# fy-vision/DiGA

Hardware: AMD Instinct MI355X
Metric: 768x768 19-class crops/sec (DiGA warm-up step) (higher is better)
Workload: dtype f32; 1 GPU; configs[1]: ResNet-101 DeepLabV2 DiGA warm-up (student + EMA teacher, KL distill), synthetic GTA5-shape 768x768, batch 8 per GPU; global_batch=8, parallelism=dp1

## Files before the change

diga_amd/_lib.py:

```python
import collections
import ctypes as C
import os

import torch

from diga_amd import config

_HERE = os.path.dirname(os.path.abspath(__file__))
LIB_PATH = os.environ.get("DIGA_LIB") or os.path.join(_HERE, "libdiga_hip.so")

if not os.path.exists(LIB_PATH):
    raise ImportError(
        f"{LIB_PATH} is missing: the DiGA hot path has no CPU fallback. "
        "Build the HIP extension first: python -m diga_amd.build")

lib = C.CDLL(LIB_PATH)

P = C.c_void_p
I64 = C.c_int64
F32 = C.c_float
INT = C.c_int
SZ = C.c_size_t

SIGNATURES = {
# ... 13 lines not shown
    "diga_ema_update_multi": (INT, [P, P, P, P, P, I64, I64, F32, F32, P]),
    "diga_sgd_momentum_multi": (INT, [P, P, P, P, P, P, P, P, I64, I64, F32, F32, INT, F32, P, P]),
    "diga_nonfinite_flag_f32": (INT, [P, I64, P, P]),
    "diga_label_hist256": (INT, [P, P, I64, I64, P]),
    "diga_classmix_paste": (INT, [P, P, P, P, P, P, P, I64, I64, I64, P]),
    "diga_centroid_softmax_weights": (INT, [P, P, P, P, I64, I64, I64, I64, P]),
    "diga_upsample_argmax_consensus": (INT, [P, P, P, P, I64, I64, I64, I64, I64, I64, P]),
    "diga_class_mean_workspace_bytes": (SZ, [I64, I64]),
    "diga_class_mean_vectors": (INT, [P, P, P, P, P, P, P, SZ, I64, I64, I64, I64, I64, I64, I64, P]),
    "diga_centroid_ema_apply": (INT, [P, P, P, P, I64, I64, I64, I64, F32, INT, INT, P]),
    "diga_confusion_matrix": (INT, [P, P, P, I64, I64, P]),
    "diga_two_scale_confusion": (INT, [P, I64, I64, P, I64, I64, P, P, P, I64, I64, I64, I64, P]),
    "diga_conv2d_nhwc_f32": (INT, [P, P, P, P] + [I64] * 17 + [P, INT, P]),
    "diga_conv2d_nhwc_f32_infer": (INT, [P, P, P, P] + [I64] * 17 + [P, INT, P]),
    "diga_conv2d_stats_floats": (SZ, [I64, I64, I64, I64]),
    "diga_conv2d_stats_chunk_rows": (INT, [I64] * 13 + [INT]),
    "diga_conv2d_epi_chunk_rows": (INT, [I64] * 13 + [INT]),
    "diga_split_bf16": (INT, [P, P, P, I64, P]),
    "diga_conv2d_nhwc_bf16x3": (INT, [P, P, P, P, P] + [I64] * 17 + [P, INT, P]),
    "diga_make_twin": (INT, [P, I64, P, I64, I64, P]),
    "diga_split_bf16_image_bytes": (SZ, [I64, I64, I64]),
    "diga_split_bf16_image": (INT, [P, P, I64, I64, I64, P]),
    "diga_conv2d_nhwc_twin": (INT, [P, P, P, P] + [I64] * 16 + [P, INT, P]),
    "diga_conv2d_nhwc_f32_opts": (INT, [P, P, P, P] + [I64] * 17 + [P, INT, P]),
    "diga_conv2d_nhwc_bf16x3_opts": (INT, [P, P, P, P, P] + [I64] * 17 + [P, INT, P]),
    "diga_conv2d_nhwc_twin_opts": (INT, [P, P, P, P] + [I64] * 16 + [P, INT, P]),
    "diga_conv2d_wgrad_workspace_bytes": (SZ, [I64] * 7),
    "diga_conv2d_wgrad_nhwc_f32": (INT, [P, P, P, P, SZ] + [I64] * 17 + [INT, P]),
    "diga_conv2d_wgrad_twin_workspace_bytes": (SZ, [I64] * 7),
    "diga_conv2d_wgrad_twin": (INT, [P, P, P, P, SZ] + [I64] * 15 + [P]),
    "diga_weight_transpose": (INT, [P, P, I64, I64, I64, P]),
    "diga_dgrad_strided_f32": (INT, [P, I64, P, P] + [I64] * 14 + [P]),
    "diga_make_triplet": (INT, [P, I64, P, I64, I64, P]),
    "diga_split_bf16x6_image_bytes": (SZ, [I64, I64, I64]),
    "diga_split_bf16x6_image": (INT, [P, P, I64, I64, I64, P]),
    "diga_conv2d_nhwc_bf16x6": (INT, [P, P, P, P] + [I64] * 16 + [P, INT, P]),
    "diga_conv2d_nhwc_bf16x6_epi": (INT, [P, P, P] + [I64] * 16 + [P, INT, P]),
    "diga_conv2d_wgrad_bf16x6_workspace_bytes": (SZ, [I64] * 7),
    "diga_conv2d_wgrad_bf16x6": (INT, [P, P, P, P, SZ] + [I64] * 15 + [P]),
    "diga_conv2d_nhwc_bf16x6_f32in": (INT, [P, I64, P, P, P] + [I64] * 16 + [P, INT, P]),
    "diga_conv2d_nhwc_bf16x6_f32in_epi": (INT, [P, I64, P, P] + [I64] * 16 + [P, INT, P]),
    "diga_infer_conv2d_nhwc_bf16x6": (INT, [P, P, P, P] + [I64] * 16 + [P, INT, P]),
    "diga_infer_conv2d_nhwc_bf16x6_f32in": (INT, [P, I64, P, P, P] + [I64] * 16 + [P, INT, P]),
    "diga_conv2d_wgrad_bf16x6_f32in": (INT, [P, I64, P, I64, P, P, SZ] + [I64] * 15 + [P]),
    "diga_conv_taps_bf16x6_f32in": (INT, [P, I64, P, P, P] + [I64] * 16 + [P, INT, P]),
    "diga_conv_taps_bf16x6_f32in_epi": (INT, [P, I64, P, P] + [I64] * 16 + [P, INT, P]),
    "diga_infer_conv_taps_bf16x6_f32in": (INT, [P, I64, P, P, P] + [I64] * 16 + [P, INT, P]),
    "diga_conv_taps_bf16x6_f32in_opts": (INT, [P, I64, P, P, P] + [I64] * 16 + [P, P, INT, P]),
    "diga_conv_window_bf16x6_plan": (INT, [I64] * 9 + [P, P, P]),
    "diga_conv_window_bf16x6_f32in": (INT, [P, I64, P, P, P] + [I64] * 14 + [P, INT, P]),
    "diga_conv_up2_bf16x6_plan": (INT, [I64] * 14 + [P, P]),
    "diga_collapse_up2_weights": (INT, [P, P] + [I64] * 6 + [P]),
    "diga_conv_up2_bf16x6_f32in": (INT, [P, I64, P, P, P, P] + [I64] * 12 + [P, INT, P]),
    "diga_conv_taps_wgrad_bf16x6_workspace_bytes": (SZ, [I64] * 7),
    "diga_conv_taps_wgrad_bf16x6_f32in": (INT, [P, I64, P, I64, P, P, SZ] + [I64] * 15 + [P]),
    "diga_wgrad_bf16x6_tile": (INT, [I64, I64, P, P]),
    "diga_wgrad_bf16x6_tiled_workspace_bytes": (SZ, [I64] * 7),
    "diga_wgrad_bf16x6_tiled_f32in": (INT, [P, I64, P, I64, P, P, SZ] + [I64] * 15 + [P]),
    "diga_im2col_nchw": (INT, [P, P] + [I64] * 11 + [P]),
    "diga_norm_workspace_bytes": (SZ, [I64, I64, I64]),
    "diga_bn_fwd": (INT, [P, I64, P, I64, P, I64, P, P, P, P, P, P, P, I64, I64, INT, INT, INT, P, F32, F32, P, SZ, P]),
    "diga_bn_eval_coefficients": (INT, [P, P, P, P, P, I64, F32, P]),
    "diga_bn_fwd_partials": (INT, [P, I64, P, I64, P, I64, P, P, P, P, P, P, P, I64, I64, INT, INT, P, F32, F32, P, I64, P, SZ, P]),
    "diga_bn_fwd_partials_resab": (INT, [P, I64, P, I64, P, I64, P, P, P, P, P, P, P, I64, I64, P, F32, F32, P, I64, P, SZ, P]),
    "diga_bn_fwd_records": (INT, [P, I64, P, I64, P, I64, P, P, P, P, P, P, P, I64, I64, INT, INT, P, F32, F32, P, P, I64, P, SZ, P]),
    "diga_bn_bwd": (INT, [P, I64, P, I64, P, I64, P, P, P, P, P, I64, P, I64, I64, I64, INT, INT, P, SZ, P]),
    "diga_bn_bwd_affine": (INT, [P, I64, P, I64, P, I64, P, P, P, P, P, I64, P, P, I64, I64, INT, P, SZ, P]),
    "diga_pyramid_sum_fwd": (INT, [P, I64, I64, P, P, I64, I64, P, I64, I64, P, I64, I64, I64, I64, P]),
    "diga_pyramid_sum_bwd": (INT, [P, I64, I64, P, I64, I64, I64, I64, P]),
    "diga_pyramid_sum_fwd3": (INT, [P, I64, I64, P, P, P, P, P, I64, I64, P]),
    "diga_pyramid_sum_bwd3": (INT, [P, I64, I64, P, P, P, I64, I64, P]),
    "diga_bn_bwd_partials": (INT, [P, I64, P, I64, P, P, P, P, I64, I64, I64, INT, P, I64, P, SZ, P]),
    "diga_conv2d_nhwc_f32_epi": (INT, [P, P, P] + [I64] * 17 + [P, INT, P]),
    "diga_conv2d_winograd_workspace_bytes": (SZ, [I64] * 7),
    "diga_conv2d_winograd_tile_table_bytes": (SZ, [I64] * 5),
    "diga_conv2d_winograd_tile_table": (INT, [P] + [I64] * 5 + [P]),
    "diga_conv2d_winograd_stats_records": (SZ, [I64] * 6),
    "diga_conv2d_winograd_stats_floats": (SZ, [I64] * 6),
    "diga_conv2d_winograd_f32": (INT, [P, P, P, P, P, SZ] + [I64] * 9 + [INT, P, P, INT, P]),
    "diga_conv2d_winograd_f32_opts": (INT, [P, P, P, P, P, SZ] + [I64] * 9 + [P, P, INT, P]),
    "diga_conv_winograd_bf16x6_opts": (INT, [P, P, P, P, P, SZ] + [I64] * 9 + [P, P, INT, P]),
    "diga_conv2d_winograd_f32_epi": (INT, [P, P, P, P, SZ] + [I64] * 9 + [INT, P, P, INT, P]),
    "diga_conv2d_winograd_f32_infer": (INT, [P, P, P, P, P, SZ] + [I64] * 9 + [P, P, INT, P]),
    "diga_conv2d_wgrad_winograd_workspace_bytes": (SZ, [I64] * 7 + [INT]),
    "diga_conv2d_wgrad_winograd_f32": (INT, [P, P, P, P, P, SZ] + [I64] * 9 + [P, P]),
    "diga_conv2d_winograd_v_floats": (SZ, [I64] * 6),
    "diga_conv2d_winograd_f32_keep": (INT, [P, P, P, P, P, P, SZ] + [I64] * 9 + [P, P, INT, P]),
    "diga_gemm_batched_bf16x6_f32in": (INT, [P, I64, I64, I64, P, I64, P, P]),
    "diga_wgrad_batched_bf16x6_workspace_bytes": (SZ, [I64] * 4),
    "diga_wgrad_batched_bf16x6_f32in": (INT, [P, P, P, P, SZ] + [I64] * 4 + [P]),
    "diga_conv2d_winograd_bf16x6_workspace_bytes": (SZ, [I64] * 7),
    "diga_conv2d_winograd_bf16x6": (INT, [P, P, P, P, P, P, SZ] + [I64] * 9 + [INT, P, P, P, INT, P]),
    "diga_infer_conv2d_winograd_bf16x6": (INT, [P, P, P, P, P, SZ] + [I64] * 9 + [P, P, INT, P]),
    "diga_conv2d_wgrad_winograd_bf16x6_workspace_bytes": (SZ, [I64] * 7 + [INT]),
    "diga_conv2d_wgrad_winograd_bf16x6": (INT, [P, P, P, P, P, SZ] + [I64] * 9 + [P, P]),
    "diga_conv2d_nhwc_bf16x3_epi": (INT, [P, P, P, P] + [I64] * 17 + [P, INT, P]),
    "diga_conv2d_nhwc_twin_epi": (INT, [P, P, P] + [I64] * 16 + [P, INT, P]),
    "diga_gn_fwd": (INT, [P, I64, P, I64, P, P, P, P, P, I64, I64, I64, I64, INT, F32, P, SZ, P]),
    "diga_gn_bwd": (INT, [P, I64, P, I64, P, I64, P, P, P, P, P, I64, P, P, I64, I64, I64, I64, P, SZ, P]),
    "diga_avgpool_nhwc": (INT, [P, I64, P, I64, I64, I64, P, SZ, P]),
    "diga_colsum_nhwc": (INT, [P, I64, P, I64, I64, P, SZ, P]),
    "diga_small_linear_fwd": (INT, [P, P, P, P, I64, I64, I64, INT, P]),
    "diga_small_linear_bwd": (INT, [P, P, P, P, P, P, P, P, I64, I64, I64, INT, P]),
    "diga_channel_affine": (INT, [P, I64, P, I64, P, P, I64, I64, I64, P]),
    "diga_channel_dot": (INT, [P, I64, P, I64, P, I64, I64, I64, P, SZ, P]),
    "diga_maxpool3x3s2_fwd": (INT, [P, P, P, I64, I64, I64, I64, I64, I64, P]),
    "diga_maxpool3x3s2_bwd": (INT, [P, P, P, I64, I64, I64, I64, I64, I64, P]),
    "diga_color_aug_view": (INT, [P, P, P, P, I64, I64, I64, F32, P, P, P]),
    "diga_ocr_workspace_bytes": (SZ, [I64, I64, I64, I64]),
    "diga_ocr_region_fwd": (INT, [P, I64, P, I64, P, P, I64, I64, I64, I64, P, SZ, P]),
    "diga_ocr_region_bwd": (INT, [P, I64, P, I64, P, P, P, P, I64, P, I64, I64, I64, I64, I64, P]),
    "diga_ocr_attend_fwd": (INT, [P, I64, P, P, P, I64, P, I64, I64, I64, I64, I64, F32, P]),
    "diga_ocr_attend_bwd": (INT, [P, I64, P, P, P, P, I64, P, I64, P, P, I64, I64, I64, I64, I64, F32, P, SZ, P]),
    "diga_mit_gemm_nt": (INT, [P, I64, P, I64, P, P, I64, INT, P, I64, P, I64, INT, F32, I64, I64, I64, P]),
    "diga_mit_gemm_tn_workspace_bytes": (SZ, [I64, I64, I64]),
    "diga_mit_gemm_tn": (INT, [P, I64, P, I64, P, P, F32, INT, P, SZ, I64, I64, I64, P]),
    "diga_mit_colsum_workspace_bytes": (SZ, [I64, I64]),
    "diga_mit_colsum": (INT, [P, I64, P, F32, INT, P, SZ, I64, I64, P]),
    "diga_mit_cast_transpose": (INT, [P, P, P, I64, I64, P]),
    "diga_mit_weight_prep_multi": (INT, [P, P, I64, I64, P]),
    "diga_mit_cast_scale": (INT, [P, P, I64, F32, P]),
    "diga_mit_row_scale": (INT, [P, P, P, I64, I64, I64, P]),
    "diga_mit_layernorm_fwd": (INT, [P, I64, P, P, P, P, I64, P, P, I64, I64, F32, P]),
    "diga_mit_layernorm_bwd_workspace_bytes": (SZ, [I64, I64]),
    "diga_mit_layernorm_bwd": (INT, [P, INT, I64, F32, P, I64, P, P, P, P, I64, P, P, I64, P, P, F32, INT, P, SZ, I64, I64, P]),
    "diga_mit_dwconv_gelu_fwd": (INT, [P, P, P, P, P, I64, I64, I64, I64, P]),
    "diga_mit_dwconv_bwd_workspace_bytes": (SZ, [I64, I64, I64]),
    "diga_mit_dwconv_gelu_bwd": (INT, [P, P, P, P, P, P, P, P, F32, INT, P, SZ, I64, I64, I64, I64, P]),
    "diga_mit_im2col": (INT, [P, INT, P] + [I64] * 11 + [P]),
    "diga_mit_col2im": (INT, [P, P, INT, F32] + [I64] * 11 + [P]),
    "diga_mit_attention_fwd": (INT, [P, I64, P, I64, P, I64, P, I64, I64, I64, I64, F32, P]),
    "diga_mit_attention_bwd_workspace_bytes": (SZ, [I64, I64, I64, I64]),
    "diga_mit_attention_bwd": (INT, [P, I64, P, I64, P, P, I64, P, P, P, P, SZ, I64, I64, I64, I64, F32, P]),
    "diga_prof_enable": (INT, [INT]),
    "diga_prof_reset": (INT, []),
    "diga_prof_query": (INT, [INT, P, P]),
    "diga_prof_query_work": (INT, [INT, P]),
}

class ConvOptions(C.Structure):
    _fields_ = [("reflect_pad", INT), ("upsample_shift", INT), ("activation", INT)]


class MitWeightPrep(C.Structure):
    _fields_ = [("src", P), ("out_a", P), ("out_b", P), ("Co", INT), ("Ci", INT), ("RS", INT), ("Kp", INT), ("mode", INT),
                ("tiles_k", INT)]


class BwdEpilogue(C.Structure):
    _fields_ = [("addend", P), ("addend_ld", I64), ("mask_y", P), ("mask_ld", I64), ("x", P), ("x_ld", I64),
                ("relu_ab", P), ("mean", P), ("invstd", P), ("partials", P), ("mask_bits", P), ("mask_bits_ld", I64)]


class InferEpilogue(C.Structure):
    _fields_ = [("ab", P), ("residual", P), ("residual_ld", I64), ("relu", INT)]


PROF_TAGS = ["ce2d", "distill", "upsample_loss", "ema", "sgd", "classmix_hist", "classmix_paste",
             "centroid_weights", "consensus", "class_means", "centroid_apply", "conv_fwd", "conv_bwd_data",
             "conv_bwd_weight", "norm", "elementwise", "mit_gemm", "mit_wgrad", "mit_attn_fwd", "mit_attn_bwd", "mit_norm",
             "mit_dwconv", "mit_misc"]


def prof_query(tag):
    n, ms = C.c_int64(0), C.c_double(0.0)
    call("diga_prof_query", PROF_TAGS.index(tag), C.byref(n), C.byref(ms))
    return n.value, ms.value

def prof_work(tag):
    w = C.c_double(0.0)
    call("diga_prof_query_work", PROF_TAGS.index(tag), C.byref(w))
    return w.value


for _name, (_res, _args) in SIGNATURES.items():
    _fn = getattr(lib, _name)
    _fn.restype = _res
    _fn.argtypes = _args


CONV_MATH_F32, CONV_MATH_BF16X3, CONV_MATH_BF16X6 = 0, 1, 2


def set_conv_math(mode, exact=None):
    mode = {"f32": 0, "bf16x3": 1, "bf16x6": 2}.get(mode, mode)
    if mode not in (CONV_MATH_F32, CONV_MATH_BF16X3, CONV_MATH_BF16X6):
        raise ValueError(f"conv math must be 0 / 'f32', 1 / 'bf16x3' or 2 / 'bf16x6', not {mode!r}")
    if exact is not None:
        if exact and mode != CONV_MATH_F32:
            raise ValueError("exact=True belongs to the fp32 arithmetic")
        config.active().winograd_max_tile = 2 if exact else config.active().winograd_default_max_tile
    config.active().conv_math = int(mode)


def get_conv_math():
    return config.active().conv_math


def last_error():
    return lib.diga_last_error_string().decode("utf-8", "replace")


def call(name, *args):
    rc = getattr(lib, name)(*args)
    if rc != 0:
        raise RuntimeError(f"{name} failed (code {rc}): {last_error()}")


def stream():
    return C.c_void_p(torch.cuda.current_stream().cuda_stream)


def ptr(t):
    return C.c_void_p(0) if t is None else C.c_void_p(t.data_ptr())


def require_gpu(*tensors):
    for t in tensors:
        if t is not None and not t.is_cuda:
            raise RuntimeError(
                "diga_amd ops run on the GPU only (HIP kernels, no CPU fallback); got a "
                f"{t.device} tensor")


def contiguous(t, dtype=None):
    if t is None:
        return None
    if dtype is not None and t.dtype != dtype:
        t = t.to(dtype)
    return t if t.is_contiguous() else t.contiguous()

# ... 86 lines not shown
```

diga_amd/config.py:

```python
import contextlib
import dataclasses
import os
from dataclasses import dataclass


def _flag(name, default):
    v = os.environ.get(name)
    if v is None:
        return default
    return v not in ("0", "", "false", "False")


@dataclass
class StepConfig:
    teacher_stream: bool = True
    teacher_offset: str = "layer1"
    wgrad_stream: bool = True
    wgrad_hold: int = 4
    wgrad_hold_batch: int = 4
    c4_overlap: int = 2
    c4_overlap_gloo: bool = False
    step_graph: bool = False
    graph_fork_teacher: bool = True
    graph_fork_wgrad: bool = True
    centroid_exchange: str = "allgather"
    conv_math: int = 0
    x6_split: str = "pass"
    x6_winograd: bool = False
    x6_taps: bool = False
    x6_opts: bool = False
    x6_window: bool = False
    x6_up2: bool = False
    x6_wgrad_tile: str = "wide"
    winograd: bool = True
    winograd_ratio: float = 0.62
    winograd_default_max_tile: int = 6
    winograd_max_tile: int = 6
    winograd_keep_v: bool = True
    winograd_stats: bool = True
    keep_v_max_gb: float = 8.0
    keep_v_min_device_gb: float = 160.0
    conv_twin: str = "3"
    twin_only: bool = True
    twin_conv3: str = "1"
    relu_bits: bool = True
    fuse_bwd: bool = True
    junction_chain: bool = True
    fold_downsample_bn: bool = True
    fold_eval_bn: bool = False
    fold_eval_bn_x6: bool = False
    ddp_bucket_mb: int = 25
    ddp_grad_views: bool = True
    ddp_overlap: bool = True
    ddp_single_rank: bool = False
    mit_loss_scale: float = 1024.0

    @classmethod
    def from_env(cls):
        e = os.environ.get
        c = cls()
        c.teacher_stream = _flag("DIGA_TEACHER_STREAM", c.teacher_stream)
        c.teacher_offset = e("DIGA_TEACHER_OFFSET", c.teacher_offset)
        c.wgrad_stream = _flag("DIGA_WGRAD_STREAM", c.wgrad_stream)
        c.wgrad_hold = int(e("DIGA_WGRAD_HOLD", c.wgrad_hold))
        c.wgrad_hold_batch = int(e("DIGA_WGRAD_HOLD_BATCH", c.wgrad_hold_batch))
        c.c4_overlap = int(e("DIGA_C4_OVERLAP", c.c4_overlap))
        c.c4_overlap_gloo = _flag("DIGA_C4_OVERLAP_GLOO", c.c4_overlap_gloo)
        c.step_graph = _flag("DIGA_STEP_GRAPH", c.step_graph)
        c.graph_fork_teacher = _flag("DIGA_GRAPH_FORK_TEACHER", c.graph_fork_teacher)
        c.graph_fork_wgrad = _flag("DIGA_GRAPH_FORK_WGRAD", c.graph_fork_wgrad)
        c.centroid_exchange = e("DIGA_CENTROID_EXCHANGE", c.centroid_exchange)
        c.conv_math = {"bf16x3": 1, "1": 1, "bf16x6": 2, "2": 2}.get(e("DIGA_CONV_MATH", ""), 0)
        c.x6_split = e("DIGA_X6_SPLIT", c.x6_split)
        c.x6_winograd = _flag("DIGA_X6_WINOGRAD", c.x6_winograd)
        c.x6_taps = _flag("DIGA_X6_TAPS", c.x6_taps)
        c.x6_opts = _flag("DIGA_X6_OPTS", c.x6_opts)
        c.x6_window = _flag("DIGA_X6_WINDOW", c.x6_window)
        c.x6_up2 = _flag("DIGA_X6_UP2", c.x6_up2)
        c.x6_wgrad_tile = e("DIGA_X6_WGRAD_TILE", c.x6_wgrad_tile)
        c.winograd = _flag("DIGA_CONV_WINOGRAD", c.winograd)
        c.winograd_ratio = float(e("DIGA_CONV_WINOGRAD_RATIO", c.winograd_ratio))
        c.winograd_default_max_tile = c.winograd_max_tile = int(e("DIGA_CONV_WINOGRAD_TILE", c.winograd_default_max_tile))
        c.winograd_keep_v = _flag("DIGA_WINOGRAD_KEEP_V", c.winograd_keep_v)
        c.winograd_stats = _flag("DIGA_WINOGRAD_STATS", c.winograd_stats)
        c.keep_v_max_gb = float(e("DIGA_WINOGRAD_KEEP_V_MAX_GB", c.keep_v_max_gb))
        c.keep_v_min_device_gb = float(e("DIGA_WINOGRAD_KEEP_V_MIN_DEVICE_GB", c.keep_v_min_device_gb))
        c.conv_twin = e("DIGA_CONV_TWIN", c.conv_twin)
        c.twin_only = _flag("DIGA_TWIN_ONLY", c.twin_only)
        c.twin_conv3 = e("DIGA_TWIN_CONV3", c.twin_conv3)
        c.relu_bits = _flag("DIGA_RELU_BITS", c.relu_bits)
        c.fuse_bwd = _flag("DIGA_FUSE_BWD", c.fuse_bwd)
        c.junction_chain = _flag("DIGA_JUNCTION_CHAIN", c.junction_chain)
        c.fold_downsample_bn = _flag("DIGA_FOLD_DOWNSAMPLE_BN", c.fold_downsample_bn)
        c.fold_eval_bn = _flag("DIGA_FOLD_EVAL_BN", c.fold_eval_bn)
        c.fold_eval_bn_x6 = _flag("DIGA_FOLD_EVAL_BN_X6", c.fold_eval_bn_x6)
        c.ddp_bucket_mb = int(e("DIGA_DDP_BUCKET_MB", c.ddp_bucket_mb))
        c.ddp_grad_views = _flag("DIGA_DDP_GRAD_VIEWS", c.ddp_grad_views)
        c.ddp_overlap = _flag("DIGA_DDP_OVERLAP", c.ddp_overlap)
        c.ddp_single_rank = _flag("DIGA_DDP_SINGLE_RANK", c.ddp_single_rank)
        c.mit_loss_scale = float(e("DIGA_MIT_LOSS_SCALE", c.mit_loss_scale))
        c.validate()
        return c

    def validate(self):
        if self.centroid_exchange not in ("allgather", "allreduce"):
            raise ValueError(f"centroid_exchange must be 'allgather' or 'allreduce', not {self.centroid_exchange!r}")
        if self.c4_overlap not in (0, 1, 2):
            raise ValueError(f"c4_overlap must be 0, 1 or 2, not {self.c4_overlap!r}")
        if self.wgrad_hold < 0:
            raise ValueError(f"wgrad_hold must be >= 0, not {self.wgrad_hold!r}")
        if self.conv_math not in (0, 1, 2):
            raise ValueError(f"conv_math must be 0 (fp32), 1 (split bf16) or 2 (bf16x6), not {self.conv_math!r}")
        if self.x6_split not in ("pass", "loader"):
            raise ValueError(f"x6_split must be 'pass' or 'loader', not {self.x6_split!r}")
        if not isinstance(self.x6_winograd, bool):
            raise ValueError(f"x6_winograd must be a bool, not {self.x6_winograd!r}")
        if not isinstance(self.x6_taps, bool):
            raise ValueError(f"x6_taps must be a bool, not {self.x6_taps!r}")
        if not isinstance(self.x6_opts, bool):
            raise ValueError(f"x6_opts must be a bool, not {self.x6_opts!r}")
        if not isinstance(self.x6_window, bool):
            raise ValueError(f"x6_window must be a bool, not {self.x6_window!r}")
        if not isinstance(self.x6_up2, bool):
            raise ValueError(f"x6_up2 must be a bool, not {self.x6_up2!r}")
        if self.x6_wgrad_tile not in ("wide", "fit"):
            raise ValueError(f"x6_wgrad_tile must be 'wide' or 'fit', not {self.x6_wgrad_tile!r}")
        if not isinstance(self.fold_eval_bn, bool):
            raise ValueError(f"fold_eval_bn must be a bool, not {self.fold_eval_bn!r}")
        if not isinstance(self.fold_eval_bn_x6, bool):
            raise ValueError(f"fold_eval_bn_x6 must be a bool, not {self.fold_eval_bn_x6!r}")
        if self.winograd_max_tile not in (2, 4, 6):
            raise ValueError(f"winograd_max_tile must be 2, 4 or 6, not {self.winograd_max_tile!r}")
        return self

    def replace(self, **fields):
        return dataclasses.replace(self, **fields).validate()

    def serial_streams(self):
        return self.replace(teacher_stream=False, wgrad_stream=False, c4_overlap=0)


DEFAULTS = StepConfig.from_env()
_stack = [DEFAULTS]


def active():
    return _stack[-1]


@contextlib.contextmanager
def use(cfg):
    _stack.append(cfg)
    try:
        yield cfg
    finally:
        _stack.pop()


@contextlib.contextmanager
def override(**fields):
    with use(active().replace(**fields)) as cfg:
        yield cfg
```

diga_amd/csrc/conv.hip:

```cpp
#include <stdlib.h>
#include <string.h>

#include <algorithm>
#include <type_traits>
#include <atomic>

#include "common.h"
#include "conv_call.h"

namespace diga {

using f32x16 = __attribute__((ext_vector_type(16))) float;
using f32x4nt = __attribute__((ext_vector_type(4))) float;

__device__ __forceinline__ void store4_stream(float* p, float x, float y, float z, float w) {
#if defined(DIGA_PROBE_NOSTORE)
    if (x == 1.2345e38f) *p = y + z + w;
#elif defined(DIGA_PROBE_PLAINSTORE)
    *reinterpret_cast<float4*>(p) = make_float4(x, y, z, w);
#else
    __builtin_nontemporal_store((f32x4nt){x, y, z, w}, reinterpret_cast<f32x4nt*>(p));
#endif
}

constexpr int kBK = 32;

struct ConvArgs {
    const float* in;
    const float* wgt;
    const uint16_t* wgt_hi;
    const uint16_t* wgt_lo;
    const unsigned char* wgt_img;
    const float* bias;
    float* out;
    float* stats;
    int N, Hi, Wi, Cin, in_ld;
    int Ho, Wo, Cout, out_ld;
    int R, S, sy, sx;
    int oy0, ox0, ody, odx;
    int M, tiles_m, tiles_n;
    int all_inside;
    const float* e_add;
    const float* e_masky;
    const unsigned char* e_maskbits;
    const float* e_x;
    const float* e_relu_ab;
    const float* e_mean;
    const float* e_invstd;
    float* e_partials;
    int e_add_ld, e_masky_ld, e_x_ld, e_maskbits_ld;
    int pad_reflect;
    int up_shift;
    int act;
    int wb_tiles = 0;
    int64_t wb_stride = 0;
    const float* i_ab = nullptr;
    const float* i_res = nullptr;
    int i_res_ld = 0;
    int i_relu = 0;
};

__device__ __forceinline__ bool map_tap(const ConvArgs& a, int iy, int ix, int& py, int& px) {
    const int Hl = a.Hi << a.up_shift, Wl = a.Wi << a.up_shift;
    bool ok = (unsigned)iy < (unsigned)Hl && (unsigned)ix < (unsigned)Wl;
    if (a.pad_reflect) {
        iy = iy < 0 ? -iy : (iy >= Hl ? 2 * (Hl - 1) - iy : iy);
        ix = ix < 0 ? -ix : (ix >= Wl ? 2 * (Wl - 1) - ix : ix);
        ok = true;
    }
    py = min(max(iy, 0), Hl - 1) >> a.up_shift;
    px = min(max(ix, 0), Wl - 1) >> a.up_shift;
    return ok;
}

__device__ __forceinline__ int xcd_remap(int orig, int nwg) {
    const int xcd = orig & 7, q = nwg >> 3, r = nwg & 7;
    return (xcd < r ? xcd * (q + 1) : r * (q + 1) + (xcd - r) * q) + (orig >> 3);
}

template <int TM, int TN, bool EPI = false, int NTHR = 256, bool INF = false, int TAG = 0>
__device__ __forceinline__ void drain_stage(const float* stage_in, const ConvArgs& a, int m0, int n0, int t, int tile_m,
                                            bool active = true);

template <int TM, int TN, bool EPI = false, bool INF = false>
__device__ __forceinline__ void epilogue_tile(f32x16 (&acc)[TM][TN], float* __restrict__ stage, const ConvArgs& a,
                                              int m0, int n0, int wm, int wn, int lane, int t, int tile_m) {
    constexpr int BN = 64 * TN, LDS_LD = BN + 4;
    const int li = lane & 31, lh = lane >> 5;
#pragma unroll
    for (int j = 0; j < TN; ++j)
#pragma unroll
// ... 2020 lines not shown
            nx = nx == 2 ? 0 : nx + 1;
        }
        return;
    }

    const int wm = wv >> 1, wn = wv & 1;
    f32x16 acc[2][2];
#pragma unroll
    for (int i = 0; i < 2; ++i)
#pragma unroll
        for (int j = 0; j < 2; ++j)
#pragma unroll
            for (int e = 0; e < 16; ++e) acc[i][j][e] = 0.f;
    const int li = lane & 31, lh = lane >> 5;
    int offa[2], offb[2];
#pragma unroll
    for (int i = 0; i < 2; ++i) {
        offa[i] = lh * A_ROW + (((wm * 64 + i * 32 + li) * 4) ^ (lh << 7));
        offb[i] = A_BYTES + lh * B_ROW + (((wn * 64 + i * 32 + li) * 4) ^ (lh << 7));
    }

    __builtin_amdgcn_s_barrier();
    int cur = 0;
    for (int ks = 0; ks < ksteps; ++ks) {
        const unsigned char* St = smem_b + cur * STAGE;
        float av[2][2], bv[2][2];
        auto frag = [&](int kk, int set) {
#pragma unroll
            for (int i = 0; i < 2; ++i) av[set][i] = *reinterpret_cast<const float*>(St + offa[i] + kk * A_ROW);
#pragma unroll
            for (int j = 0; j < 2; ++j) bv[set][j] = *reinterpret_cast<const float*>(St + offb[j] + kk * B_ROW);
        };
        frag(0, 0);
#pragma unroll
        for (int kk = 0; kk < kBK; kk += 2) {
            const int set = (kk >> 1) & 1;
            if (kk + 2 < kBK) frag(kk + 2, set ^ 1);
            __builtin_amdgcn_sched_group_barrier(0x100, 4, 0);
#pragma unroll
            for (int i = 0; i < 2; ++i)
#pragma unroll
                for (int j = 0; j < 2; ++j)
                    acc[i][j] = __builtin_amdgcn_mfma_f32_32x32x2f32(av[set][i], bv[set][j], acc[i][j], 0, 0, 0);
            __builtin_amdgcn_sched_group_barrier(0x008, 4, 0);
        }
        asm volatile("s_waitcnt lgkmcnt(0)" ::: "memory");
        __builtin_amdgcn_s_barrier();
        cur = cur == 2 ? 0 : cur + 1;
    }

    float* out = a.slab + (int64_t)split * a.Cout * RS * a.Cin;
#pragma unroll
    for (int j = 0; j < 2; ++j) {
        const int c = c0 + wn * 64 + j * 32 + li;
#pragma unroll
        for (int i = 0; i < 2; ++i) {
#pragma unroll
            for (int e = 0; e < 16; ++e) {
                const int k = k0 + wm * 64 + i * 32 + (e & 3) + 8 * (e >> 2) + 4 * lh;
                out[((int64_t)k * RS + tap) * a.Cin + c] = acc[i][j][e];
            }
        }
    }
}

__global__ __launch_bounds__(256) void slab_reduce_kernel(const float* __restrict__ slab, float* __restrict__ dw,
                                                          int64_t n4, int splits) {
    const int64_t i = (int64_t)blockIdx.x * 256 + threadIdx.x;
    if (i >= n4) return;
    float4 s = reinterpret_cast<const float4*>(slab)[i];
    for (int k = 1; k < splits; ++k) {
        const float4 v = reinterpret_cast<const float4*>(slab)[(int64_t)k * n4 + i];
        s.x += v.x;
        s.y += v.y;
        s.z += v.z;
        s.w += v.w;
    }
    reinterpret_cast<float4*>(dw)[i] = s;
}

__global__ __launch_bounds__(256) void weight_transpose_kernel(const float* __restrict__ w, float* __restrict__ wt,
                                                               int K, int RS, int C) {
    __shared__ float tile[32][33];
    const int tap = blockIdx.z;
    const int k0 = blockIdx.y * 32, c0 = blockIdx.x * 32;
    const int tx = threadIdx.x & 31, ty = threadIdx.x >> 5;
#pragma unroll
    for (int i = 0; i < 4; ++i) {
        const int k = k0 + ty + 8 * i, c = c0 + tx;
        tile[ty + 8 * i][tx] = (k < K && c < C) ? w[((int64_t)k * RS + tap) * C + c] : 0.f;
    }
    __syncthreads();
#pragma unroll
    for (int i = 0; i < 4; ++i) {
        const int c = c0 + ty + 8 * i, k = k0 + tx;
        if (c < C && k < K) wt[((int64_t)c * RS + tap) * K + k] = tile[tx][ty + 8 * i];
    }
}

static int check_conv_common(const char* who, int64_t Cin, int64_t in_ld, int64_t out_ld, int64_t Cout,
                             const void* in, const void* w, const void* out) {
    DIGA_REQUIRE(Cin > 0 && Cin % 32 == 0, DIGA_EINVAL, "%s: Cin=%lld must be a multiple of 32", who, (long long)Cin);
    DIGA_REQUIRE(in_ld >= Cin && in_ld % 4 == 0 && out_ld >= Cout, DIGA_EINVAL, "%s: bad leading dimensions", who);
    DIGA_REQUIRE(aligned16(in) && aligned16(w), DIGA_EALIGN, "%s: pointers must be 16-byte aligned", who);
    (void)out;
    return DIGA_OK;
}

static int check_options(const diga_conv_options_t* o, const char* who) {
    if (o == nullptr) return DIGA_OK;
    DIGA_REQUIRE(o->reflect_pad >= 0 && o->reflect_pad <= 1 && o->upsample_shift >= 0 && o->upsample_shift <= 2 && o->activation >= 0 &&
                     o->activation <= 1, DIGA_EINVAL, "%s: bad options (reflect_pad 0/1, upsample_shift 0..2, activation 0/1)", who);
    return DIGA_OK;
}

static int fill_conv_args(ConvArgs& a, const ConvCall& c, const char* who, const char* who_infer) {
    a = ConvArgs{};
    a.in = static_cast<const float*>(c.in); a.wgt = c.wgt; a.wgt_hi = c.wgt_hi; a.wgt_lo = c.wgt_lo;
    a.wgt_img = static_cast<const unsigned char*>(c.wgt_img); a.bias = c.bias; a.out = c.out; a.stats = c.stats;
    a.N = (int)c.N; a.Hi = (int)c.Hi; a.Wi = (int)c.Wi; a.Cin = (int)c.Cin; a.in_ld = (int)(c.in_ld >= 0 ? c.in_ld : c.Cin);
    a.Ho = (int)c.Ho; a.Wo = (int)c.Wo; a.Cout = (int)c.Cout; a.out_ld = (int)c.out_ld;
    a.R = (int)c.R; a.S = (int)c.S; a.sy = (int)c.stride_y; a.sx = (int)c.stride_x;
    a.oy0 = (int)c.off_y0; a.ox0 = (int)c.off_x0; a.ody = (int)c.off_dy; a.odx = (int)c.off_dx;
    a.M = (int)(c.N * c.Ho * c.Wo);
    int rc = check_options(c.opts, who);
    if (rc) return rc;
    if (const diga_conv_options_t* o = c.opts) {
        a.pad_reflect = o->reflect_pad; a.up_shift = o->upsample_shift; a.act = o->activation;
    }
    const bool out4 = c.Cout % 4 == 0 && c.out_ld % 4 == 0 && aligned16(c.out) && c.stats == nullptr;
    rc = check_bwd_epilogue(c.epi, c.Cout, who, out4 && c.bias == nullptr);
    if (rc) return rc;
    if (const diga_bwd_epilogue_t* e = c.epi) {
        a.e_add = e->addend; a.e_add_ld = (int)e->addend_ld;
        a.e_masky = e->mask_y; a.e_masky_ld = (int)e->mask_ld;
        a.e_maskbits = e->mask_bits; a.e_maskbits_ld = (int)e->mask_bits_ld;
        a.e_x = e->x; a.e_x_ld = (int)e->x_ld;
        a.e_relu_ab = e->relu_ab; a.e_mean = e->mean; a.e_invstd = e->invstd; a.e_partials = e->partials;
    }
    rc = check_infer_epilogue(c.infer, c.Cout, c.out, who_infer, out4 && (c.bias == nullptr || aligned16(c.bias)));
    if (rc) return rc;
    if (const diga_infer_epilogue_t* e = c.infer) {
        a.i_ab = e->ab;
        a.i_res = e->residual;
        a.i_res_ld = e->residual ? (int)e->residual_ld : 0;
        a.i_relu = e->relu ? 1 : 0;
    }
    return DIGA_OK;
}

template <class Args>
static void launch_k(void (*kernel)(Args), unsigned grid, unsigned threads, size_t sh, hipStream_t st, const Args& a) {
    (void)hipFuncSetAttribute((const void*)kernel, hipFuncAttributeMaxDynamicSharedMemorySize, (int)sh);
    hipLaunchKernelGGL(kernel, dim3(grid), dim3(threads), sh, st, a);
}
using ConvKernel = void (*)(ConvArgs);
using WgradKernel = void (*)(WgradArgs);

struct GemmArgs {
    const float* A;
    const float* W;
    float* out;
    int M, K, Cout, tiles_m, tiles_n, wb_tiles;
    int rows_valid;
    int64_t wb_stride;
    int64_t a_ld, out_ld;
    const float* bias;
    float* stats;
    const float* i_ab = nullptr;
    const float* i_res = nullptr;
    int64_t i_res_ld = 0;
    int i_relu = 0;
};

template <bool STATS, bool BIAS, int INF = 0>
__global__ __launch_bounds__(768, 3) void gemm_f32_persistent_kernel(GemmArgs g) {
    static_assert(INF == 0 || !STATS, "no statistics next to the inference epilogue");
    constexpr int A_BYTES = 256 * 128, B_BYTES = 128 * 128, STAGE = A_BYTES + B_BYTES;
    extern __shared__ __align__(16) unsigned char smem_b[];
    const int lane = threadIdx.x & 63, wv = threadIdx.x >> 6;
// ... 868 lines not shown
```

diga_amd/csrc/winograd.hip:

```cpp
#include <type_traits>

#include "common.h"
#include "conv_call.h"

namespace diga {

int gemm_batched_f32_dma(const float* A, int64_t rows_per_batch, int batches, int64_t K, const float* W, int64_t Cout,
                         float* out, hipStream_t st, int64_t rows_valid);
size_t wgrad_batched_slab_bytes(int64_t rows, int batches, int64_t Cout, int64_t Cin);
int wgrad_batched_f32_dma(const float* Z, const float* V, float* dU, float* slab, int64_t rows, int batches, int64_t Cout,
                          int64_t Cin, hipStream_t st);
int split_image3_batched(const float* U, void* imgs, int batches, int64_t Cout, int64_t K, hipStream_t st);
bool gemm_batched_bf16x6_ok(int64_t rows_per_batch, int64_t batches, int64_t K, int64_t Cout);
int gemm_batched_bf16x6(const float* A, int64_t rows_per_batch, int batches, int64_t K, const void* imgs, int64_t Cout, float* out,
                        hipStream_t st);
bool wgrad_batched_bf16x6_ok(int64_t rows, int64_t batches, int64_t Cout, int64_t Cin);
size_t wgrad_batched_bf16x6_slab_bytes(int64_t rows, int batches, int64_t Cout, int64_t Cin);
int wgrad_batched_bf16x6(const float* Z, const float* V, float* dU, float* slab, int64_t rows, int batches, int64_t Cout, int64_t Cin,
                         hipStream_t st);

namespace wino {

struct WinoGeom {
    int N, H, W, d;
    int m;
    int tys, txs;
    int64_t T, Tp;
};

int phase_tiles(int len, int d, int m) {
    int s = 0;
    for (int a = 0; a < d; ++a) {
        const int n = len > a ? (len - a + d - 1) / d : 0;
        s += (n + m - 1) / m;
    }
    return s;
}

WinoGeom make_wino(int64_t N, int64_t H, int64_t W, int64_t d, int64_t m) {
    WinoGeom g;
    g.N = (int)N; g.H = (int)H; g.W = (int)W; g.d = (int)d; g.m = (int)m;
    g.tys = phase_tiles((int)H, (int)d, (int)m);
    g.txs = phase_tiles((int)W, (int)d, (int)m);
    g.T = N * g.tys * g.txs;
    g.Tp = ceil_div(g.T, 256) * 256;
    return g;
}
static inline int products(int64_t m) { return (int)((m + 2) * (m + 2)); }
static inline bool tile_ok(int64_t m) { return m == 2 || m == 4 || m == 6; }

__global__ __launch_bounds__(256) void wino_tiles_kernel(int4* __restrict__ tab, WinoGeom g) {
    const int64_t t = (int64_t)blockIdx.x * 256 + threadIdx.x;
    if (t >= g.Tp) return;
    if (t >= g.T) {
        tab[t] = make_int4(-1, 0, 0, 0);
        return;
    }
    const int timg = g.tys * g.txs;
    const int n = (int)(t / timg), r = (int)(t - (int64_t)n * timg);
    constexpr int kBand = 1;
    const int band = r / (kBand * g.txs), rem = r - band * kBand * g.txs;
    const int rows_in_band = min(kBand, g.tys - kBand * band);
    int Cc = rem / rows_in_band, R = kBand * band + (rem - Cc * rows_in_band);
    int a = 0, b = 0;
    for (; a < g.d; ++a) {
        const int cnt = g.H > a ? (g.H - a + g.d - 1) / g.d : 0;
        const int tl = (cnt + g.m - 1) / g.m;
        if (R < tl) break;
        R -= tl;
    }
    for (; b < g.d; ++b) {
        const int cnt = g.W > b ? (g.W - b + g.d - 1) / g.d : 0;
        const int tl = (cnt + g.m - 1) / g.m;
        if (Cc < tl) break;
        Cc -= tl;
    }
    tab[t] = make_int4(n, a + g.m * R * g.d, b + g.m * Cc * g.d, 0);
}

using f32x4nt = __attribute__((ext_vector_type(4))) float;
__device__ __forceinline__ void nt_store4(float* p, float4 v) {
    __builtin_nontemporal_store((f32x4nt){v.x, v.y, v.z, v.w}, reinterpret_cast<f32x4nt*>(p));
}
__device__ __forceinline__ float4 nt_load4(const float* p) {
    const f32x4nt v = __builtin_nontemporal_load(reinterpret_cast<const f32x4nt*>(p));
    return make_float4(v.x, v.y, v.z, v.w);
// ... 4 lines not shown

__device__ __forceinline__ float4 f4fma(float s, float4 a, float4 b) {
    return make_float4(__builtin_fmaf(s, a.x, b.x), __builtin_fmaf(s, a.y, b.y), __builtin_fmaf(s, a.z, b.z), __builtin_fmaf(s, a.w, b.w));
}
__device__ __forceinline__ float4 f4scale(float s, float4 a) { return make_float4(s * a.x, s * a.y, s * a.z, s * a.w); }
__device__ __forceinline__ float2 f4add(float2 a, float2 b) { return make_float2(a.x + b.x, a.y + b.y); }
__device__ __forceinline__ float2 f4sub(float2 a, float2 b) { return make_float2(a.x - b.x, a.y - b.y); }
__device__ __forceinline__ float2 f4fma(float s, float2 a, float2 b) { return make_float2(__builtin_fmaf(s, a.x, b.x), __builtin_fmaf(s, a.y, b.y)); }
__device__ __forceinline__ float2 f4scale(float s, float2 a) { return make_float2(s * a.x, s * a.y); }
__device__ __forceinline__ float f4add(float a, float b) { return a + b; }
__device__ __forceinline__ float f4sub(float a, float b) { return a - b; }
__device__ __forceinline__ float f4fma(float s, float a, float b) { return __builtin_fmaf(s, a, b); }
__device__ __forceinline__ float f4scale(float s, float a) { return s * a; }
__device__ __forceinline__ void nt_store4(float* p, float v) { __builtin_nontemporal_store(v, p); }
using f32x2nt = __attribute__((ext_vector_type(2))) float;
__device__ __forceinline__ void nt_store4(float* p, float2 v) {
    __builtin_nontemporal_store((f32x2nt){v.x, v.y}, reinterpret_cast<f32x2nt*>(p));
}
template <typename V> __device__ __forceinline__ V nt_loadv(const float* p);
template <> __device__ __forceinline__ float4 nt_loadv<float4>(const float* p) { return nt_load4(p); }
template <> __device__ __forceinline__ float2 nt_loadv<float2>(const float* p) {
    const f32x2nt v = __builtin_nontemporal_load(reinterpret_cast<const f32x2nt*>(p));
    return make_float2(v.x, v.y);
}
template <> __device__ __forceinline__ float nt_loadv<float>(const float* p) { return __builtin_nontemporal_load(p); }
template <typename V> __device__ __forceinline__ V vzero();
template <> __device__ __forceinline__ float vzero<float>() { return 0.f; }
template <> __device__ __forceinline__ float4 vzero<float4>() { return make_float4(0.f, 0.f, 0.f, 0.f); }
template <> __device__ __forceinline__ float2 vzero<float2>() { return make_float2(0.f, 0.f); }

#include "winograd_xforms.h"

template <int M> struct Xf;
template <> struct Xf<2> {
    template <typename V> static __device__ __forceinline__ void bt(const V* x, V* r) {
        r[0] = f4sub(x[0], x[2]);
        r[1] = f4add(x[1], x[2]);
        r[2] = f4sub(x[2], x[1]);
        r[3] = f4sub(x[1], x[3]);
    }
    template <typename V> static __device__ __forceinline__ void g(const V* x, V* r) {
        const V sum = f4add(x[0], x[2]);
        r[0] = x[0];
        r[1] = f4half(f4add(sum, x[1]));
        r[2] = f4half(f4sub(sum, x[1]));
        r[3] = x[2];
    }
    template <typename V> static __device__ __forceinline__ void at(const V* x, V* r) {
        r[0] = f4add(f4add(x[0], x[1]), x[2]);
        r[1] = f4sub(f4sub(x[1], x[2]), x[3]);
    }
    template <typename V> static __device__ __forceinline__ void a(const V* x, V* r) {
        r[0] = x[0];
        r[1] = f4add(x[0], x[1]);
        r[2] = f4sub(x[0], x[1]);
        r[3] = f4sub(vzero<V>(), x[1]);
    }
    template <typename V> static __device__ __forceinline__ void gt(const V* x, V* r) {
        const V hs = f4half(f4add(x[1], x[2])), hd = f4half(f4sub(x[1], x[2]));
        r[0] = f4add(x[0], hs);
        r[1] = hd;
        r[2] = f4add(hs, x[3]);
    }
};
template <> struct Xf<4> {
    template <typename V> static __device__ __forceinline__ void bt(const V* x, V* r) { wino4_bt(x, r); }
    template <typename V> static __device__ __forceinline__ void g(const V* x, V* r) { wino4_g(x, r); }
    template <typename V> static __device__ __forceinline__ void at(const V* x, V* r) { wino4_at(x, r); }
    template <typename V> static __device__ __forceinline__ void a(const V* x, V* r) { wino4_a(x, r); }
    template <typename V> static __device__ __forceinline__ void gt(const V* x, V* r) { wino4_gt(x, r); }
};
template <> struct Xf<6> {
    template <typename V> static __device__ __forceinline__ void bt(const V* x, V* r) { wino6_bt(x, r); }
    template <typename V> static __device__ __forceinline__ void g(const V* x, V* r) { wino6_g(x, r); }
    template <typename V> static __device__ __forceinline__ void at(const V* x, V* r) { wino6_at(x, r); }
    template <typename V> static __device__ __forceinline__ void a(const V* x, V* r) { wino6_a(x, r); }
    template <typename V> static __device__ __forceinline__ void gt(const V* x, V* r) { wino6_gt(x, r); }
};
template <int M> struct Vec;
template <> struct Vec<2> { using In = float4; using Out = float4; using Dy = float4; using Dw = float4; static constexpr int EpiLanes = 4, EpiBlocks = 3; };
template <> struct Vec<4> { using In = float4; using Out = float2; using Dy = float4; using Dw = float2; static constexpr int EpiLanes = 2, EpiBlocks = 4; };
template <> struct Vec<6> { using In = float2; using Out = float; using Dy = float2; using Dw = float2; static constexpr int EpiLanes = 2, EpiBlocks = 4; };

template <int M>
__global__ __launch_bounds__(256) void winoM_weight_kernel(const float* __restrict__ w, float* __restrict__ U, int Cout, int Cin,
                                                           int flip) {
    constexpr int A = M + 2;
    const int64_t idx = (int64_t)blockIdx.x * 256 + threadIdx.x;
    const int c4n = Cin / 4;
    if (idx >= (int64_t)Cout * c4n) return;
    const int co = (int)(idx / c4n), c = (int)(idx - (int64_t)co * c4n) * 4;
    float4 t[A][3];
#pragma unroll
    for (int s = 0; s < 3; ++s) {
        float4 g[3];
#pragma unroll
        for (int r = 0; r < 3; ++r) {
            const int rr = flip ? 2 - r : r, ss = flip ? 2 - s : s;
            g[r] = *reinterpret_cast<const float4*>(w + ((int64_t)co * 9 + rr * 3 + ss) * Cin + c);
        }
        float4 col[A];
        Xf<M>::g(g, col);
#pragma unroll
        for (int i = 0; i < A; ++i) t[i][s] = col[i];
    }
    const int64_t plane = (int64_t)Cout * Cin;
    float* o = U + (int64_t)co * Cin + c;
#pragma unroll
    for (int i = 0; i < A; ++i) {
        float4 row[A];
        Xf<M>::g(t[i], row);
#pragma unroll
        for (int j = 0; j < A; ++j) *reinterpret_cast<float4*>(o + (A * i + j) * plane) = row[j];
    }
}

template <typename V> __device__ __forceinline__ void wino_in_store(float* p, V v) { nt_store4(p, v); }
template <int M, typename V, bool REFLECT = false>
__global__ __launch_bounds__(256) void winoM_input_kernel(const float* __restrict__ x, int64_t ld, const int4* __restrict__ tab,
                                                          float* __restrict__ Vo, int64_t Tp, int C, int H, int W, int d) {
    constexpr bool reflect = REFLECT;
    constexpr int A = M + 2;
    constexpr int VW = sizeof(V) / 4;
    const int c4n = C / VW;
    const int64_t idx = (int64_t)blockIdx.x * 256 + threadIdx.x;
    if (idx >= Tp * c4n) return;
    const int64_t t = idx / c4n;
    const int c = (int)(idx - t * c4n) * VW;
    const int4 e = tab[t];
    const V z = vzero<V>();
    const int img = max(e.x, 0);
    V m[A][A];
#pragma unroll
    for (int j = 0; j < A; ++j) {
        int xx = e.z + (j - 1) * d;
        if (reflect) {
            xx = xx < 0 ? -xx : xx;
            xx = xx >= W ? 2 * (W - 1) - xx : xx;
        }
        const bool xok = e.x >= 0 && (reflect || (unsigned)xx < (unsigned)W);
        const int xc = min(max(xx, 0), W - 1);
        V p[A];
#pragma unroll
        for (int i = 0; i < A; ++i) {
            int y = e.y + (i - 1) * d;
            if (reflect) {
                y = y < 0 ? -y : y;
                y = y >= H ? 2 * (H - 1) - y : y;
            }
            const bool ok = xok && (reflect || (unsigned)y < (unsigned)H);
            const int yc = min(max(y, 0), H - 1);
            const V v = *reinterpret_cast<const V*>(x + ((int64_t)(img * H + yc) * W + xc) * ld + c);
            p[i] = ok ? v : z;
        }
        V col[A];
        Xf<M>::bt(p, col);
#pragma unroll
        for (int i = 0; i < A; ++i) m[i][j] = col[i];
    }
    float* o = Vo + t * C + c;
    const int64_t plane = Tp * C;
#pragma unroll
    for (int i = 0; i < A; ++i) {
        V row[A];
        Xf<M>::bt(m[i], row);
#pragma unroll
        for (int j = 0; j < A; ++j) wino_in_store<V>(o + (A * i + j) * plane, row[j]);
    }
}

__global__ __launch_bounds__(256) void wino_input_kernel(const float* __restrict__ x, int64_t ld, const int4* __restrict__ tab,
                                                         float* __restrict__ V, int64_t Tp, int C, int H, int W, int d) {
    const int c4n = C / 4;
    const int64_t idx = (int64_t)blockIdx.x * 256 + threadIdx.x;
    if (idx >= Tp * c4n) return;
    const int64_t t = idx / c4n;
    const int c = (int)(idx - t * c4n) * 4;
    const int4 e = tab[t];
    const float4 z = make_float4(0.f, 0.f, 0.f, 0.f);
    const int img = max(e.x, 0);
    float4 p[4][4];
#pragma unroll
    for (int i = 0; i < 4; ++i) {
        const int y = e.y + (i - 1) * d;
        const bool yok = e.x >= 0 && (unsigned)y < (unsigned)H;
        const int yc = min(max(y, 0), H - 1);
#pragma unroll
        for (int j = 0; j < 4; ++j) {
            const int xx = e.z + (j - 1) * d;
            const bool ok = yok && (unsigned)xx < (unsigned)W;
            const float4 v = *reinterpret_cast<const float4*>(x + ((int64_t)(img * H + yc) * W + min(max(xx, 0), W - 1)) * ld + c);
            p[i][j] = ok ? v : z;
        }
    }
    float4 m[4][4];
#pragma unroll
// ... 459 lines not shown
                           (int)Cout, g.H, g.W, g.d, tpb, ep);
}
template <int M, bool ADD>
static void launch_output_epi2_mask(const float* Mb, const int4* tab, float* out, int64_t out_ld, const WinoGeom& g, int64_t Cout, int64_t G,
                                    int tpb, const WinoEpi& ep, hipStream_t st) {
    if (ep.masky != nullptr) launch_output_epi2_sums<M, ADD, 1>(Mb, tab, out, out_ld, g, Cout, G, tpb, ep, st);
    else if (ep.maskbits != nullptr) launch_output_epi2_sums<M, ADD, 2>(Mb, tab, out, out_ld, g, Cout, G, tpb, ep, st);
    else if (ep.relu_ab != nullptr) launch_output_epi2_sums<M, ADD, 3>(Mb, tab, out, out_ld, g, Cout, G, tpb, ep, st);
    else launch_output_epi2_sums<M, ADD, 0>(Mb, tab, out, out_ld, g, Cout, G, tpb, ep, st);
}
template <int M>
static void launch_output_epi2_m(const float* Mb, const int4* tab, float* out, int64_t out_ld, const WinoGeom& g, int64_t Cout, int64_t G,
                                 int tpb, const WinoEpi& ep, hipStream_t st) {
    if (ep.add != nullptr) launch_output_epi2_mask<M, true>(Mb, tab, out, out_ld, g, Cout, G, tpb, ep, st);
    else launch_output_epi2_mask<M, false>(Mb, tab, out, out_ld, g, Cout, G, tpb, ep, st);
}

template <int M>
static void launch_dy_m(const float* dy, int64_t dy_ld, const int4* tab, float* Z, const WinoGeom& g, int64_t Cout, hipStream_t st) {
    using VT = typename Vec<M>::Dy;
    constexpr int VW = sizeof(VT) / 4;
    hipLaunchKernelGGL((winoM_dy_kernel<M, VT>), dim3((unsigned)ceil_div(g.Tp * (Cout / VW), 256)), dim3(256), 0, st, dy, dy_ld, tab, Z, g.Tp,
                       (int)Cout, g.H, g.W, g.d);
}
template <int M>
static void launch_dw_m(const float* dU, float* dw, int64_t Cout, int64_t Cin, hipStream_t st) {
    using VT = typename Vec<M>::Dw;
    constexpr int VW = sizeof(VT) / 4;
    hipLaunchKernelGGL((winoM_dw_kernel<M, VT>), dim3((unsigned)ceil_div(Cout * (Cin / VW), 256)), dim3(256), 0, st, dU, dw, (int)Cout, (int)Cin);
}

struct WinoWgradLayout {
    size_t tab, V, Z, dU, slab, total;
};
WinoWgradLayout wino_wgrad_layout(const WinoGeom& g, int64_t Cin, int64_t Cout, bool with_v, bool x6 = false) {
    WinoWgradLayout l;
    size_t o = 0;
    l.tab = o; o += (size_t)g.Tp * sizeof(int4);
    l.V = o; o += with_v ? (size_t)products(g.m) * g.Tp * Cin * sizeof(float) : 0;
    l.Z = o; o += (size_t)products(g.m) * g.Tp * Cout * sizeof(float);
    l.dU = o; o += (size_t)products(g.m) * Cout * Cin * sizeof(float);
    l.slab = o; o += x6 ? wgrad_batched_bf16x6_slab_bytes(g.Tp, products(g.m), Cout, Cin)
                        : wgrad_batched_slab_bytes(g.Tp, products(g.m), Cout, Cin);
    l.total = o + 64;
    return l;
}

struct WinoLayout {
    size_t tab, U, img, V, M, total;
};
WinoLayout wino_layout(const WinoGeom& g, int64_t Cin, int64_t Cout, bool x6 = false) {
    WinoLayout l;
    size_t o = 0;
    l.tab = o; o += (size_t)g.Tp * sizeof(int4);
    l.U = o; o += (size_t)products(g.m) * Cout * Cin * sizeof(float);
    l.img = o; o += x6 ? (size_t)products(g.m) * diga_split_bf16x6_image_bytes(Cout, 1, Cin) : 0;
    l.V = o; o += (size_t)products(g.m) * g.Tp * Cin * sizeof(float);
    l.M = o; o += (size_t)products(g.m) * g.Tp * Cout * sizeof(float);
    l.total = o + 64;
    return l;
}

struct WinoShape {
    void* workspace = nullptr;
    size_t workspace_bytes = 0;
    int64_t N = 0, H = 0, W = 0, Cin = 0, Cout = 0, dilation = 0, tile = 0;
    const void* tile_table = nullptr;
    void* stream = nullptr;
    bool x6 = false;
};
#define DIGA_FILL_WINO(c_)                                                                                              \
    do {                                                                                                               \
        (c_).workspace = workspace; (c_).workspace_bytes = workspace_bytes; (c_).N = N; (c_).H = H; (c_).W = W; (c_).Cin = Cin;     \
        (c_).Cout = Cout; (c_).dilation = dilation; (c_).tile = tile; (c_).tile_table = tile_table; (c_).stream = stream;          \
    } while (0)
struct WinoCall : WinoShape {
    const float* in = nullptr;
    const float* wgt = nullptr;
    const float* bias = nullptr;
    float* out = nullptr;
    int64_t in_ld = 0, out_ld = 0;
    int flip = 0, reflect = 0, prof_tag = 0;
    float* v_keep = nullptr;
    float* stats = nullptr;
    const diga_bwd_epilogue_t* epi = nullptr;
    const diga_infer_epilogue_t* infer = nullptr;
};
struct WinoWgradCall : WinoShape {
    const float* dy = nullptr;
    const float* x = nullptr;
    const float* v_kept = nullptr;
    float* dw = nullptr;
    int64_t x_ld = 0, dy_ld = 0;
};

}
}

using namespace diga;
using namespace diga::wino;

extern "C" size_t diga_conv2d_winograd_workspace_bytes(int64_t N, int64_t H, int64_t W, int64_t Cin, int64_t Cout, int64_t dilation, int64_t tile) {
    if (N <= 0 || H <= 0 || W <= 0 || Cin <= 0 || Cout <= 0 || dilation <= 0 || !tile_ok(tile)) return 0;
    return wino_layout(make_wino(N, H, W, dilation, tile), Cin, Cout).total;
}

static int winograd_conv(const WinoCall& c) {
    const float *in = c.in, *wgt = c.wgt, *bias = c.bias;
    float *out = c.out, *stats = c.stats;
    const int64_t N = c.N, H = c.H, W = c.W, Cin = c.Cin, in_ld = c.in_ld, Cout = c.Cout, out_ld = c.out_ld, dilation = c.dilation, tile = c.tile;
    const int flip = c.flip, reflect = c.reflect;
    const bool x6 = c.x6;
    const diga_bwd_epilogue_t* epi = c.epi;
    const diga_infer_epilogue_t* inf = c.infer;
    const void* tile_table = c.tile_table;
    DIGA_REQUIRE(!inf || ((tile == 4 || tile == 6) && !flip && !epi && !stats && !reflect), DIGA_EINVAL,
                 "conv2d_winograd_infer: the inference epilogue comes with the plain forward of 4x4 / 6x6 tiles");
    DIGA_REQUIRE(!reflect || (tile != 2 && !flip && !epi && dilation < H && dilation < W), DIGA_EINVAL,
                 "conv2d_winograd: reflection padding comes with the forward of 4x4 / 6x6 tiles (pad < H, W)");
    DIGA_REQUIRE(in && wgt && out && c.workspace, DIGA_EINVAL, "conv2d_winograd: null pointer");
    DIGA_REQUIRE(N > 0 && H > 0 && W > 0 && dilation > 0 && dilation < 4096, DIGA_EINVAL, "conv2d_winograd: bad shape");
    DIGA_REQUIRE(tile_ok(tile), DIGA_EINVAL, "conv2d_winograd: tile must be 2, 4 or 6 (F(2x2,3x3) / F(4x4,3x3) / F(6x6,3x3))");
    DIGA_REQUIRE(Cin % 32 == 0 && Cout % 4 == 0 && Cout > 64 && in_ld >= Cin && in_ld % 4 == 0 && out_ld >= Cout && out_ld % 4 == 0,
                 DIGA_EINVAL, "conv2d_winograd: Cin %% 32, Cout %% 4 (> 64) and leading dimensions %% 4 required");
    DIGA_REQUIRE(aligned16(in) && aligned16(wgt) && aligned16(out) && aligned16(c.workspace) && (!bias || aligned16(bias)), DIGA_EALIGN,
                 "conv2d_winograd: pointers must be 16-byte aligned");
    DIGA_REQUIRE(N * H * W < (1ll << 31), DIGA_EINVAL, "conv2d_winograd: too many pixels");
    const WinoGeom g = make_wino(N, H, W, dilation, tile);
    const int P = products(tile);
    DIGA_REQUIRE(x6 || P * g.Tp / 256 < 32768, DIGA_EINVAL, "conv2d_winograd: too many tiles for one launch");
    DIGA_REQUIRE(!x6 || gemm_batched_bf16x6_ok(g.Tp, P, Cin, Cout), DIGA_EINVAL,
                 "conv2d_winograd_bf16x6: products * padded tiles and the GEMM's tile count must stay below 2^31");
    const WinoLayout l = wino_layout(g, Cin, Cout, x6);
    DIGA_REQUIRE(c.workspace_bytes >= l.total, DIGA_EWORKSPACE, "conv2d_winograd: workspace too small (%zu < %zu)", c.workspace_bytes, l.total);
    DIGA_REQUIRE(!stats || (epi == nullptr && tile != 2 && aligned16(stats)), DIGA_EINVAL,
                 "conv2d_winograd: statistics come with the forward output transform of 4x4 / 6x6 tiles (16-byte aligned buffer)");
    DIGA_REQUIRE(!tile_table || aligned16(tile_table), DIGA_EALIGN, "conv2d_winograd: tile_table must be 16-byte aligned");
    char* ws = static_cast<char*>(c.workspace);
    const int4* tab = tile_table != nullptr ? static_cast<const int4*>(tile_table) : reinterpret_cast<const int4*>(ws + l.tab);
    float* U = reinterpret_cast<float*>(ws + l.U);
    float* V = c.v_keep != nullptr ? c.v_keep : reinterpret_cast<float*>(ws + l.V);
    float* Mb = reinterpret_cast<float*>(ws + l.M);
    hipStream_t st = (hipStream_t)c.stream;
    ProfScope prof(c.prof_tag == DIGA_PROF_CONV_BWD_DATA ? DIGA_PROF_CONV_BWD_DATA : DIGA_PROF_CONV_FWD, st,
                   2.0 * (double)(N * H * W) * (double)Cout * 9.0 * (double)Cin);
    if (tile_table == nullptr)
        hipLaunchKernelGGL(wino_tiles_kernel, dim3((unsigned)ceil_div(g.Tp, 256)), dim3(256), 0, st, reinterpret_cast<int4*>(ws + l.tab), g);
    with_tile(tile, [&](auto m) { launch_weight_m<decltype(m)::value>(wgt, U, Cout, Cin, flip, st); });
    launch_input(tile, in, in_ld, tab, V, g.Tp, Cin, H, W, dilation, st, reflect);
    int rc;
    if (x6) {
        void* imgs = ws + l.img;
        split_image3_batched(U, imgs, P, Cout, Cin, st);
        rc = gemm_batched_bf16x6(V, g.Tp, P, Cin, imgs, Cout, Mb, st);
    } else {
        rc = gemm_batched_f32_dma(V, g.Tp, P, Cin, U, Cout, Mb, st, g.T);
    }
    if (rc) return rc;
    if (epi == nullptr && stats != nullptr) {
        with_tile<4>(tile, [&](auto m) { launch_output_stats_m<decltype(m)::value>(Mb, tab, bias, out, out_ld, g, Cout, stats, st); });
    } else if (epi == nullptr && inf != nullptr) {
        with_tile<4>(tile, [&](auto m) { launch_output_infer_m<decltype(m)::value>(Mb, tab, bias, out, out_ld, g, Cout, *inf, st); });
    } else if (epi == nullptr) {
        with_tile(tile, [&](auto m) { launch_output_m<decltype(m)::value>(Mb, tab, bias, out, out_ld, g, Cout, st); });
    } else {
        WinoEpi ep;
        ep.add = epi->addend; ep.add_ld = epi->addend_ld;
        ep.masky = epi->mask_y; ep.masky_ld = epi->mask_ld;
        ep.maskbits = epi->mask_bits; ep.maskbits_ld = epi->mask_bits_ld;
        ep.x = epi->x; ep.x_ld = epi->x_ld;
        ep.relu_ab = epi->relu_ab; ep.mean = epi->mean; ep.invstd = epi->invstd; ep.partials = epi->partials;
        const int64_t G = ceil_div(N * H * W, 128);
        const int tpb = (int)ceil_div(g.T, G);
        with_tile(tile, [&](auto m) { launch_output_epi2_m<decltype(m)::value>(Mb, tab, out, out_ld, g, Cout, G, tpb, ep, st); });
    }
    return launch_status(x6 ? (reflect ? "diga_conv_winograd_bf16x6_opts" : "diga_conv2d_winograd_bf16x6") : "diga_conv2d_winograd_f32");
}

extern "C" size_t diga_conv2d_winograd_tile_table_bytes(int64_t N, int64_t H, int64_t W, int64_t dilation, int64_t tile) {
    if (N <= 0 || H <= 0 || W <= 0 || dilation <= 0 || !tile_ok(tile)) return 0;
    return (size_t)make_wino(N, H, W, dilation, tile).Tp * sizeof(int4);
}

extern "C" int diga_conv2d_winograd_tile_table(void* table, int64_t N, int64_t H, int64_t W, int64_t dilation, int64_t tile, void* stream) {
    DIGA_REQUIRE(table && aligned16(table), DIGA_EINVAL, "conv2d_winograd_tile_table: null / unaligned table");
    DIGA_REQUIRE(N > 0 && H > 0 && W > 0 && dilation > 0 && dilation < 4096 && tile_ok(tile) && N * H * W < (1ll << 31), DIGA_EINVAL,
                 "conv2d_winograd_tile_table: bad shape / tile");
    const WinoGeom g = make_wino(N, H, W, dilation, tile);
    hipLaunchKernelGGL(wino_tiles_kernel, dim3((unsigned)ceil_div(g.Tp, 256)), dim3(256), 0, (hipStream_t)stream, static_cast<int4*>(table), g);
    return launch_status("diga_conv2d_winograd_tile_table");
}

extern "C" size_t diga_conv2d_winograd_stats_records(int64_t N, int64_t H, int64_t W, int64_t Cout, int64_t dilation, int64_t tile) {
    if (N <= 0 || H <= 0 || W <= 0 || Cout <= 0 || dilation <= 0 || (tile != 4 && tile != 6)) return 0;
    return (size_t)stats_plan(make_wino(N, H, W, dilation, tile), Cout).records;
}

extern "C" size_t diga_conv2d_winograd_stats_floats(int64_t N, int64_t H, int64_t W, int64_t Cout, int64_t dilation, int64_t tile) {
    const size_t r = diga_conv2d_winograd_stats_records(N, H, W, Cout, dilation, tile);
    return r * 3 * (size_t)Cout + r;
}

extern "C" int diga_conv2d_winograd_f32(const float* in, const float* wgt, const float* bias, float* out, void* workspace,
                                        size_t workspace_bytes, int64_t N, int64_t H, int64_t W, int64_t Cin, int64_t in_ld,
                                        int64_t Cout, int64_t out_ld, int64_t dilation, int64_t tile, int flip, float* stats_partial,
                                        const void* tile_table, int prof_tag, void* stream) {
    WinoCall c;
    DIGA_FILL_WINO(c);
    c.in = in; c.in_ld = in_ld; c.wgt = wgt; c.bias = bias; c.out = out; c.out_ld = out_ld; c.flip = flip; c.stats = stats_partial;
    c.prof_tag = prof_tag;
    return winograd_conv(c);
}

extern "C" int diga_conv2d_winograd_f32_opts(const float* in, const float* wgt, const float* bias, float* out, void* workspace,
                                             size_t workspace_bytes, int64_t N, int64_t H, int64_t W, int64_t Cin, int64_t in_ld,
                                             int64_t Cout, int64_t out_ld, int64_t dilation, int64_t tile, const diga_conv_options_t* opts,
                                             const void* tile_table, int prof_tag, void* stream) {
    DIGA_REQUIRE(opts != nullptr, DIGA_EINVAL, "conv2d_winograd_opts: null options");
    DIGA_REQUIRE(opts->upsample_shift == 0 && opts->activation == 0, DIGA_EINVAL,
                 "conv2d_winograd_opts: only reflect_pad is folded on the Winograd path (upsampling / tanh: the direct `_opts` kernels)");
    WinoCall c;
    DIGA_FILL_WINO(c);
    c.in = in; c.in_ld = in_ld; c.wgt = wgt; c.bias = bias; c.out = out; c.out_ld = out_ld; c.reflect = opts->reflect_pad ? 1 : 0;
    c.prof_tag = prof_tag;
    return winograd_conv(c);
}

extern "C" int diga_conv2d_winograd_f32_infer(const float* in, const float* wgt, const float* bias, float* out, void* workspace,
                                              size_t workspace_bytes, int64_t N, int64_t H, int64_t W, int64_t Cin, int64_t in_ld,
                                              int64_t Cout, int64_t out_ld, int64_t dilation, int64_t tile,
                                              const diga_infer_epilogue_t* infer, const void* tile_table, int prof_tag, void* stream) {
    DIGA_REQUIRE(infer != nullptr, DIGA_EINVAL, "conv2d_winograd_infer: null epilogue descriptor");
    const int rc = check_infer_epilogue(infer, Cout, out, "conv2d_winograd_infer");
    if (rc) return rc;
    WinoCall c;
    DIGA_FILL_WINO(c);
    c.in = in; c.in_ld = in_ld; c.wgt = wgt; c.bias = bias; c.out = out; c.out_ld = out_ld; c.infer = infer; c.prof_tag = prof_tag;
    return winograd_conv(c);
}

extern "C" size_t diga_conv2d_winograd_v_floats(int64_t N, int64_t H, int64_t W, int64_t Cin, int64_t dilation, int64_t tile) {
    if (N <= 0 || H <= 0 || W <= 0 || Cin <= 0 || dilation <= 0 || !tile_ok(tile)) return 0;
    return (size_t)products(tile) * make_wino(N, H, W, dilation, tile).Tp * Cin;
}

extern "C" int diga_conv2d_winograd_f32_keep(const float* in, const float* wgt, const float* bias, float* out, float* v_keep,
                                             void* workspace, size_t workspace_bytes, int64_t N, int64_t H, int64_t W, int64_t Cin,
                                             int64_t in_ld, int64_t Cout, int64_t out_ld, int64_t dilation, int64_t tile,
                                             float* stats_partial, const void* tile_table, int prof_tag, void* stream) {
    DIGA_REQUIRE(v_keep != nullptr && aligned16(v_keep), DIGA_EINVAL, "conv2d_winograd_keep: v_keep must be a 16-byte aligned buffer");
    WinoCall c;
    DIGA_FILL_WINO(c);
    c.in = in; c.in_ld = in_ld; c.wgt = wgt; c.bias = bias; c.out = out; c.out_ld = out_ld; c.v_keep = v_keep; c.stats = stats_partial;
    c.prof_tag = prof_tag;
    return winograd_conv(c);
}

extern "C" int diga_conv2d_winograd_f32_epi(const float* in, const float* wgt, float* out, void* workspace, size_t workspace_bytes,
                                            int64_t N, int64_t H, int64_t W, int64_t Cin, int64_t in_ld, int64_t Cout,
                                            int64_t out_ld, int64_t dilation, int64_t tile, int flip, const diga_bwd_epilogue_t* e,
                                            const void* tile_table, int prof_tag, void* stream) {
    DIGA_REQUIRE(e != nullptr, DIGA_EINVAL, "conv2d_winograd_epi: null epilogue descriptor");
    const int rc = check_bwd_epilogue(e, Cout, "conv2d_winograd_epi");
    if (rc) return rc;
    WinoCall c;
    DIGA_FILL_WINO(c);
    c.in = in; c.in_ld = in_ld; c.wgt = wgt; c.out = out; c.out_ld = out_ld; c.flip = flip; c.epi = e; c.prof_tag = prof_tag;
    return winograd_conv(c);
}

extern "C" size_t diga_conv2d_wgrad_winograd_workspace_bytes(int64_t N, int64_t H, int64_t W, int64_t Cin, int64_t Cout,
                                                             int64_t dilation, int64_t tile, int v_kept) {
    if (N <= 0 || H <= 0 || W <= 0 || Cin <= 0 || Cout <= 0 || dilation <= 0 || Cout % 256 != 0 || Cin % 128 != 0 || !tile_ok(tile)) return 0;
    return wino_wgrad_layout(make_wino(N, H, W, dilation, tile), Cin, Cout, v_kept == 0).total;
}

static int winograd_wgrad(const WinoWgradCall& c) {
    const float *dy = c.dy, *x = c.x, *v_kept = c.v_kept;
    float* dw = c.dw;
    void* workspace = c.workspace;
    const int64_t N = c.N, H = c.H, W = c.W, Cin = c.Cin, x_ld = c.x_ld, Cout = c.Cout, dy_ld = c.dy_ld, dilation = c.dilation, tile = c.tile;
    const void* tile_table = c.tile_table;
    const bool x6 = c.x6;
    DIGA_REQUIRE(!tile_table || aligned16(tile_table), DIGA_EALIGN, "conv2d_wgrad_winograd: tile_table must be 16-byte aligned");
    DIGA_REQUIRE(dy && (x || v_kept) && dw && workspace, DIGA_EINVAL, "conv2d_wgrad_winograd: null pointer");
    DIGA_REQUIRE(!v_kept || aligned16(v_kept), DIGA_EALIGN, "conv2d_wgrad_winograd: v_kept must be 16-byte aligned");
    DIGA_REQUIRE(N > 0 && H > 0 && W > 0 && dilation > 0 && dilation < 4096 && N * H * W < (1ll << 31) && tile_ok(tile),
                 DIGA_EINVAL, "conv2d_wgrad_winograd: bad shape / tile");
    DIGA_REQUIRE(Cout % 256 == 0 && Cin % 128 == 0 && x_ld >= Cin && x_ld % 4 == 0 && dy_ld >= Cout && dy_ld % 4 == 0, DIGA_EINVAL,
                 "conv2d_wgrad_winograd: Cout %% 256, Cin %% 128 and leading dimensions %% 4 required");
    DIGA_REQUIRE(aligned16(dy) && (!x || aligned16(x)) && aligned16(dw) && aligned16(workspace), DIGA_EALIGN,
                 "conv2d_wgrad_winograd: pointers must be 16-byte aligned");
    const WinoGeom g = make_wino(N, H, W, dilation, tile);
    DIGA_REQUIRE(!x6 || wgrad_batched_bf16x6_ok(g.Tp, products(tile), Cout, Cin), DIGA_EINVAL,
                 "conv2d_wgrad_winograd_bf16x6: padded tiles and the GEMM's block count must stay below 2^31");
    const WinoWgradLayout l = wino_wgrad_layout(g, Cin, Cout, v_kept == nullptr, x6);
    DIGA_REQUIRE(c.workspace_bytes >= l.total, DIGA_EWORKSPACE, "conv2d_wgrad_winograd: workspace too small (%zu < %zu)", c.workspace_bytes,
                 l.total);
    char* ws = static_cast<char*>(workspace);
    const int4* tab = tile_table != nullptr ? static_cast<const int4*>(tile_table) : reinterpret_cast<const int4*>(ws + l.tab);
    const float* V = v_kept != nullptr ? v_kept : reinterpret_cast<float*>(ws + l.V);
    float* Z = reinterpret_cast<float*>(ws + l.Z);
    float* dU = reinterpret_cast<float*>(ws + l.dU);
    float* slab = reinterpret_cast<float*>(ws + l.slab);
    hipStream_t st = (hipStream_t)c.stream;
    ProfScope prof(DIGA_PROF_CONV_BWD_WEIGHT, st, 2.0 * (double)(N * H * W) * (double)Cout * 9.0 * (double)Cin);
    if (tile_table == nullptr)
        hipLaunchKernelGGL(wino_tiles_kernel, dim3((unsigned)ceil_div(g.Tp, 256)), dim3(256), 0, st, reinterpret_cast<int4*>(ws + l.tab), g);
    if (v_kept == nullptr)
        launch_input(tile, x, x_ld, tab, reinterpret_cast<float*>(ws + l.V), g.Tp, Cin, H, W, dilation, st);
    with_tile(tile, [&](auto m) { launch_dy_m<decltype(m)::value>(dy, dy_ld, tab, Z, g, Cout, st); });
    int rc = x6 ? wgrad_batched_bf16x6(Z, V, dU, slab, g.Tp, products(tile), Cout, Cin, st)
                : wgrad_batched_f32_dma(Z, V, dU, slab, g.Tp, products(tile), Cout, Cin, st);
    if (rc) return rc;
    with_tile(tile, [&](auto m) { launch_dw_m<decltype(m)::value>(dU, dw, Cout, Cin, st); });
    return launch_status(x6 ? "diga_conv2d_wgrad_winograd_bf16x6" : "diga_conv2d_wgrad_winograd_f32");
}

extern "C" int diga_conv2d_wgrad_winograd_f32(const float* dy, const float* x, const float* v_kept, float* dw, void* workspace,
                                              size_t workspace_bytes, int64_t N, int64_t H, int64_t W, int64_t Cin, int64_t x_ld,
                                              int64_t Cout, int64_t dy_ld, int64_t dilation, int64_t tile, const void* tile_table,
                                              void* stream) {
    WinoWgradCall c;
    DIGA_FILL_WINO(c);
    c.dy = dy; c.dy_ld = dy_ld; c.x = x; c.x_ld = x_ld; c.v_kept = v_kept; c.dw = dw;
    return winograd_wgrad(c);
}

extern "C" size_t diga_conv2d_winograd_bf16x6_workspace_bytes(int64_t N, int64_t H, int64_t W, int64_t Cin, int64_t Cout,
                                                              int64_t dilation, int64_t tile) {
    if (N <= 0 || H <= 0 || W <= 0 || Cin <= 0 || Cin % 32 != 0 || Cout <= 64 || Cout % 4 != 0 || dilation <= 0 || dilation >= 4096 ||
        !tile_ok(tile) || N * H * W >= (1ll << 31))
        return 0;
    const WinoGeom g = make_wino(N, H, W, dilation, tile);
    if (!gemm_batched_bf16x6_ok(g.Tp, products(tile), Cin, Cout)) return 0;
    return wino_layout(g, Cin, Cout, true).total;
}

extern "C" int diga_conv2d_winograd_bf16x6(const float* in, const float* wgt, const float* bias, float* out, float* v_keep,
                                           void* workspace, size_t workspace_bytes, int64_t N, int64_t H, int64_t W, int64_t Cin,
                                           int64_t in_ld, int64_t Cout, int64_t out_ld, int64_t dilation, int64_t tile, int flip,
                                           float* stats_partial, const diga_bwd_epilogue_t* e, const void* tile_table, int prof_tag,
                                           void* stream) {
    DIGA_REQUIRE(!v_keep || aligned16(v_keep), DIGA_EALIGN, "conv2d_winograd_bf16x6: v_keep must be 16-byte aligned");
    DIGA_REQUIRE(!v_keep || (!flip && !e), DIGA_EINVAL, "conv2d_winograd_bf16x6: v_keep comes with the forward (flip = 0, no epilogue)");
    DIGA_REQUIRE(!e || (!bias && !stats_partial), DIGA_EINVAL, "conv2d_winograd_bf16x6: a backward epilogue takes no bias and no statistics");
    const int rc = check_bwd_epilogue(e, Cout, "conv2d_winograd_bf16x6");
    if (rc) return rc;
    WinoCall c;
    DIGA_FILL_WINO(c);
// ... 53 lines not shown
```

diga_amd/model/conv.py:

```python
import ctypes
import os
import sys
from typing import NamedTuple

import torch
import torch.nn as nn

_pkg = os.path.dirname(os.path.dirname(os.path.abspath(__file__)))
if os.path.dirname(_pkg) not in sys.path:
    sys.path.append(os.path.dirname(_pkg))
from diga_amd import _lib, config

_TAG_FWD, _TAG_BWD_DATA = _lib.PROF_TAGS.index("conv_fwd"), _lib.PROF_TAGS.index("conv_bwd_data")


def _pad_to(c, q=32):
    return (c + q - 1) // q * q


def _pad_last(t, c_to):
    c = t.shape[-1]
    if c == c_to:
        return t
    out = t.new_zeros(t.shape[:-1] + (c_to,))
    out[..., :c] = t
    return out



def _bias_grad(gy):
    k = gy.shape[-1]
    ld = gy.stride(2)
    m = gy.shape[0] * gy.shape[1] * gy.shape[2]
    dense = gy.stride(3) == 1 and gy.stride(1) == gy.shape[2] * ld and gy.stride(0) == gy.shape[1] * gy.stride(1)
    if not dense or ((k % 4 != 0 or ld % 4 != 0) and k > 64):
        return gy.sum(dim=(0, 1, 2))
    out = torch.empty(k, dtype=torch.float32, device=gy.device)
    ws = _lib.workspace(_lib.lib.diga_norm_workspace_bytes(m, 1, k), gy.device, "norm")
    _lib.call("diga_colsum_nhwc", _lib.ptr(gy), ld, _lib.ptr(out), m, k, _lib.ptr(ws), ws.numel(), _lib.stream())
    return out


def _use_twin(cin, k, taps, shared):
    mode = config.active().conv_twin
    if mode == "0" or cin % 32 != 0 or k <= 64:
        return False
    return mode == "1" or taps > 1 or shared


def _use_x6(cin, r, s):
    return r == 1 and s == 1 and cin % 32 == 0


def _x6_taps():
    return _lib.get_conv_math() == 2 and config.active().x6_taps


def _x6_opts():
    return _lib.get_conv_math() == 2 and config.active().x6_opts


def _taps_ok(cin, r, s, copt):
    return 1 < r * s <= 64 and cin % 32 == 0 and (not copt or _x6_opts())


def _x6_window(hi, wi, cin, k, r, s, doff, shift):
    if not (_x6_taps() and config.active().x6_window) or doff[0] < 1 or doff[1] < 1:
        return False
    th, tw, cols = ctypes.c_int(0), ctypes.c_int(0), ctypes.c_int(0)
    return _lib.lib.diga_conv_window_bf16x6_plan(hi, wi, cin, k, r, s, doff[0], doff[1], shift, ctypes.byref(th), ctypes.byref(tw),
                                                 ctypes.byref(cols)) == 1


def _x6_up2(hi, wi, cin, k, ho, wo, r, s, off0, doff, opts):
    if not (_x6_opts() and config.active().x6_up2):
        return False
    rc, sc = ctypes.c_int(0), ctypes.c_int(0)
    return _lib.lib.diga_conv_up2_bf16x6_plan(hi, wi, cin, k, ho, wo, r, s, off0[0], off0[1], doff[0], doff[1], int(opts[1]),
                                              int(opts[0]), ctypes.byref(rc), ctypes.byref(sc)) == 1


def _x6_fit(kp, cp):
    if _lib.get_conv_math() != 2 or config.active().x6_wgrad_tile != "fit":
        return False
    bm, bn = ctypes.c_int(0), ctypes.c_int(0)
    _lib.call("diga_wgrad_bf16x6_tile", kp, cp, ctypes.byref(bm), ctypes.byref(bn))
    return (bm.value, bn.value) != (256, 128)


def _x6_loader():
    return config.active().x6_split == "loader"


def _nhwc_ld(t):
# ... 254 lines not shown
            ld = rn.shape[3]
        e.residual, e.residual_ld = _lib.ptr(rn), ld
    e.relu = 1 if relu else 0
    return e, (ab, rn)


def _make_split(src, ld, rows, ch, triplet):
    out = torch.empty(rows * ch * (6 if triplet else 4), dtype=torch.uint8, device=src.device)
    _lib.call("diga_make_triplet" if triplet else "diga_make_twin", _lib.ptr(src), ld, _lib.ptr(out), rows, ch, _lib.stream())
    return out


_ENTRY = {
    ("x6ls", ""): "diga_conv2d_nhwc_bf16x6_f32in", ("x6ls", "epi"): "diga_conv2d_nhwc_bf16x6_f32in_epi",
    ("x6ls", "infer"): "diga_infer_conv2d_nhwc_bf16x6_f32in",
    ("x6rs", ""): "diga_conv_taps_bf16x6_f32in", ("x6rs", "epi"): "diga_conv_taps_bf16x6_f32in_epi",
    ("x6rs", "infer"): "diga_infer_conv_taps_bf16x6_f32in", ("x6rs", "opts"): "diga_conv_taps_bf16x6_f32in_opts",
    ("x6win", ""): "diga_conv_window_bf16x6_f32in", ("x6win", "opts"): "diga_conv_window_bf16x6_f32in",
    ("x6up2", "opts"): "diga_conv_up2_bf16x6_f32in",
    ("x6", ""): "diga_conv2d_nhwc_bf16x6", ("x6", "epi"): "diga_conv2d_nhwc_bf16x6_epi", ("x6", "infer"): "diga_infer_conv2d_nhwc_bf16x6",
    ("twin", ""): "diga_conv2d_nhwc_twin", ("twin", "epi"): "diga_conv2d_nhwc_twin_epi", ("twin", "opts"): "diga_conv2d_nhwc_twin_opts",
    ("bf16x3", ""): "diga_conv2d_nhwc_bf16x3", ("bf16x3", "epi"): "diga_conv2d_nhwc_bf16x3_epi",
    ("bf16x3", "opts"): "diga_conv2d_nhwc_bf16x3_opts",
    ("f32", ""): "diga_conv2d_nhwc_f32", ("f32", "epi"): "diga_conv2d_nhwc_f32_epi", ("f32", "opts"): "diga_conv2d_nhwc_f32_opts",
    ("f32", "infer"): "diga_conv2d_nhwc_f32_infer",
    ("winograd", ""): "diga_conv2d_winograd_f32", ("winograd", "epi"): "diga_conv2d_winograd_f32_epi",
    ("winograd", "infer"): "diga_conv2d_winograd_f32_infer", ("winograd", "keep"): "diga_conv2d_winograd_f32_keep",
    ("winograd_reflect", "opts"): "diga_conv2d_winograd_f32_opts",
}
_WINOGRAD_X6 = "diga_conv2d_winograd_bf16x6"
_WINOGRAD_X6_INFER = "diga_infer_conv2d_winograd_bf16x6"
_WINOGRAD_X6_OPTS = "diga_conv_winograd_bf16x6_opts"


def _up2_phase_images(w_krsc, hi, wi, ho, wo, off0, opts):
    k, r, s, cin = w_krsc.shape
    rc, sc = ctypes.c_int(0), ctypes.c_int(0)
    if _lib.lib.diga_conv_up2_bf16x6_plan(hi, wi, cin, k, ho, wo, r, s, off0[0], off0[1], 1, 1, int(opts[1]), int(opts[0]),
                                          ctypes.byref(rc), ctypes.byref(sc)) != 1:
        raise RuntimeError("DigaConv2d: diga_conv_up2_bf16x6_plan does not take a call planned as 'x6up2'")
    rs = rc.value * sc.value
    wc = torch.empty((4, k, rc.value, sc.value, cin), dtype=torch.float32, device=w_krsc.device)
    _lib.call("diga_collapse_up2_weights", _lib.ptr(w_krsc), _lib.ptr(wc), k, r, s, cin, off0[0], off0[1], _lib.stream())
    size = _lib.lib.diga_split_bf16x6_image_bytes(k, rs, cin)
    imgs = torch.empty(4 * size, dtype=torch.uint8, device=w_krsc.device)
    for ph in range(4):
        _lib.call("diga_split_bf16x6_image", _lib.ptr(wc[ph]), _lib.ptr(imgs[ph * size:]), k, rs, cin, _lib.stream())
    return wc, imgs


def _operands(path, x, w_krsc, twin_box, up2=None):
    n, hi, wi, cin = x.shape
    k, r, s, _ = w_krsc.shape
    if path.family in ("x6ls", "x6rs", "x6win", "x6up2"):
        split, ld = None, _nhwc_ld(x)
        if ld is None:
            x, ld = x.contiguous(), cin
        act = [_lib.ptr(x), ld]
    elif path.family in ("x6", "twin"):
        split = twin_box[0] if twin_box is not None else None
        if split is None:
            split = _make_split(x if x.is_contiguous() else x.contiguous(), cin, n * hi * wi, cin, path.family == "x6")
            if twin_box is not None:
                twin_box[0] = split
        act = [_lib.ptr(split)]
    if path.family in ("x6ls", "x6rs", "x6win", "x6up2", "x6", "twin"):
        size, fill = ((_lib.lib.diga_split_bf16_image_bytes, "diga_split_bf16_image") if path.family == "twin" else
                      (_lib.lib.diga_split_bf16x6_image_bytes, "diga_split_bf16x6_image"))
        img = torch.empty(size(k, r * s, cin), dtype=torch.uint8, device=x.device)
        _lib.call(fill, _lib.ptr(w_krsc), _lib.ptr(img), k, r * s, cin, _lib.stream())
        if path.family == "x6up2":
            wc, imgs = _up2_phase_images(w_krsc, hi, wi, *up2)
            return act + [_lib.ptr(img), _lib.ptr(imgs)], (x, split, img, wc, imgs), split
        return act + [_lib.ptr(img)], (x, split, img), split
    if path.family == "bf16x3":
        nel = w_krsc.numel()
        w_hi = torch.empty(nel, dtype=torch.int16, device=w_krsc.device)
        w_lo = torch.empty(nel, dtype=torch.int16, device=w_krsc.device)
        _lib.call("diga_split_bf16", _lib.ptr(w_krsc), _lib.ptr(w_hi), _lib.ptr(w_lo), nel, _lib.stream())
        return [_lib.ptr(x), _lib.ptr(w_hi), _lib.ptr(w_lo)], (w_hi, w_lo), None
    return [_lib.ptr(x), _lib.ptr(w_krsc)], (), None


def _winograd_launch(path, x, w_krsc, bias, out, d, flip, tag, stats, struct, keep_v):
    n, hi, wi, cin = x.shape
    k, tile = out.shape[3], path.tile
    size = _lib.lib.diga_conv2d_winograd_bf16x6_workspace_bytes if path.x6w else _lib.lib.diga_conv2d_winograd_workspace_bytes
    ws = _lib.workspace(size(n, hi, wi, cin, k, d, tile), x.device, "winograd")
    tab = _tile_table(n, hi, wi, d, tile, x.device)
    variant, vk = path.variant, None
    if variant == "keep":
        vk = keep_v[0] = _alloc_keep_v(_lib.lib.diga_conv2d_winograd_v_floats(n, hi, wi, cin, d, tile), x.device)
        if vk is None:
            variant = ""
    lead = [_lib.ptr(x), _lib.ptr(w_krsc)] + ([] if variant == "epi" and not path.x6w else [_lib.ptr(bias)]) + [_lib.ptr(out)]
    shape = (_lib.ptr(ws), ws.numel(), n, hi, wi, cin, x.stride(2), k, out.stride(2), d, tile)
    if path.x6w and variant in ("infer", "opts"):
        _lib.call(_WINOGRAD_X6_INFER if variant == "infer" else _WINOGRAD_X6_OPTS, *lead, *shape, struct, _lib.ptr(tab), tag, _lib.stream())
        return
    if path.x6w:
        _lib.call(_WINOGRAD_X6, *lead, _lib.ptr(vk), *shape, flip, _lib.ptr(stats), struct, _lib.ptr(tab), tag, _lib.stream())
        return
    if variant == "keep":
        lead.append(_lib.ptr(vk))
    _lib.call(_ENTRY[(path.family, variant)], *lead, *shape, *((flip,) if variant in ("", "epi") else ()),
              struct if struct is not None else _lib.ptr(stats), _lib.ptr(tab), tag, _lib.stream())


def _conv_launch(x, w_krsc, bias, out, stride, off0, doff, tag, stats=None, twin_box=None, must_twin=False, epi=None,
                 opts=None, keep_v=None, x6_ok=True, infer=None, path=None):
    n, hi, wi, cin = x.shape
    _, ho, wo, k = out.shape
    _, r, s, _ = w_krsc.shape
    if path is None:
        path = _plan(n, hi, wi, cin, k, r, s, stride, off0, doff, ho, wo, tag, None if stats is None else "chunks", epi is not None,
                     opts, infer is not None, twin_box is not None, must_twin, x6_ok)
    struct = inf_held = None
    if path.variant == "epi":
        struct = ctypes.byref(epi)
    elif path.variant == "opts":
        struct = ctypes.byref(_lib.ConvOptions(int(opts[0]), int(opts[1]), int(opts[2])))
    elif path.variant == "infer":
        inf, inf_held = _infer_epilogue(infer, out)
        struct = ctypes.byref(inf)
    direct = 2.0 * n * ho * wo * k * r * s * cin
    _log_path(tag, path.arith)
    if path.flops:
        _log_flops("conv_bwd_data" if tag == _TAG_BWD_DATA else "conv_fwd", direct, direct * path.ratio)
    if path.family in ("winograd", "winograd_reflect"):
        _winograd_launch(path, x, w_krsc, bias, out, abs(doff[0]), 1 if doff[0] < 0 else 0, tag, stats, struct, keep_v)
        return None
    lead, held, split = _operands(path, x, w_krsc, twin_box, (ho, wo, off0, opts))
    if path.family == "x6up2":
        _lib.call(_ENTRY[(path.family, path.variant)], *lead, _lib.ptr(bias), _lib.ptr(out), n, hi, wi, cin, ho, wo, k, out.stride(2), r, s,
                  off0[0], off0[1], struct, tag, _lib.stream())
        return split
    if path.family == "x6win":
        _lib.call(_ENTRY[(path.family, path.variant)], *lead, _lib.ptr(bias), _lib.ptr(out), n, hi, wi, cin, ho, wo, k, out.stride(2), r, s,
                  off0[0], off0[1], doff[0], doff[1], struct, tag, _lib.stream())
        return split
    _lib.call(_ENTRY[(path.family, path.variant)], *lead, *(() if path.variant == "epi" else (_lib.ptr(bias),)), _lib.ptr(out),
              n, hi, wi, cin, *((x.stride(2),) if path.family in ("bf16x3", "f32") else ()), ho, wo, k, out.stride(2), r, s,
              stride[0], stride[1], off0[0], off0[1], doff[0], doff[1],
              *((_lib.ptr(stats),) if (path.family, path.variant) == ("x6rs", "opts") else ()),
              struct if struct is not None else _lib.ptr(stats), tag, _lib.stream())
    return split


_WGRAD = {
    "x6ls": ("diga_conv2d_wgrad_bf16x6_f32in", _lib.lib.diga_conv2d_wgrad_bf16x6_workspace_bytes),
    "x6rs": ("diga_conv_taps_wgrad_bf16x6_f32in", _lib.lib.diga_conv_taps_wgrad_bf16x6_workspace_bytes),
    "x6": ("diga_conv2d_wgrad_bf16x6", _lib.lib.diga_conv2d_wgrad_bf16x6_workspace_bytes),
    "twin": ("diga_conv2d_wgrad_twin", _lib.lib.diga_conv2d_wgrad_twin_workspace_bytes),
    "f32": ("diga_conv2d_wgrad_nhwc_f32", _lib.lib.diga_conv2d_wgrad_workspace_bytes),
}
_WGRAD_FIT = ("diga_wgrad_bf16x6_tiled_f32in", _lib.lib.diga_wgrad_bf16x6_tiled_workspace_bytes)
_WGRAD_WINOGRAD = {
    False: ("diga_conv2d_wgrad_winograd_f32", _lib.lib.diga_conv2d_wgrad_winograd_workspace_bytes),
    True: ("diga_conv2d_wgrad_winograd_bf16x6", _lib.lib.diga_conv2d_wgrad_winograd_bf16x6_workspace_bytes),
}


def _wgrad_launch(path, gy, x, dwp, r, s, stride, padding, dilation, splits=None, wino_v=None):
    n, hi, wi, cp = x.shape
    _, ho, wo, kp = gy.shape
    _log_path("wgrad", path.arith)
    if path.flops:
        direct = 2.0 * n * ho * wo * kp * r * s * cp
        _log_flops("conv_bwd_weight", direct, direct * path.ratio)
    if path.family == "winograd":
        name, size = _WGRAD_WINOGRAD[path.x6w]
        ws = _lib.workspace(size(n, hi, wi, cp, kp, dilation[0], path.tile, 1 if wino_v is not None else 0), x.device, "winograd_wgrad")
        tab = _tile_table(n, hi, wi, dilation[0], path.tile, x.device)
        _lib.call(name, _lib.ptr(gy), _lib.ptr(x), _lib.ptr(wino_v), _lib.ptr(dwp), _lib.ptr(ws), ws.numel(), n, hi, wi, cp, x.stride(2),
                  kp, gy.stride(2), dilation[0], path.tile, _lib.ptr(tab), _lib.stream())
        return
    name, size = _WGRAD_FIT if path.fit else _WGRAD[path.family]
    ws = _lib.workspace(size(n, ho, wo, kp, cp, r, s), x.device, "wgrad")
    f32 = path.family == "f32"
    if path.family in ("x6ls", "x6rs"):
        lead = (_lib.ptr(gy), gy.stride(2), _lib.ptr(x), x.stride(2))
    else:
        lead = (_lib.ptr(gy), _lib.ptr(x)) if f32 else (_lib.ptr(splits[0]), _lib.ptr(splits[1]))
    _lib.call(name, *lead, _lib.ptr(dwp), _lib.ptr(ws), ws.numel(), n, hi, wi, cp, *((x.stride(2),) if f32 else ()), ho, wo, kp,
              *((gy.stride(2),) if f32 else ()), r, s, stride[0], stride[1], -padding[0], -padding[1], dilation[0], dilation[1],
              *((path.math,) if f32 else ()), _lib.stream())


class _Call(NamedTuple):
    stride: tuple = (1, 1)
    padding: tuple = (0, 0)
    dilation: tuple = (1, 1)
    stats: object = None
    uses: object = None
    twin_box: object = None
    x_is_twin: bool = False
    dy_is_twin: bool = False
    bn_box: object = None
    opts: object = None
    chain: object = None
    infer: object = None


class _StemConvFn(torch.autograd.Function):

    @staticmethod
    def forward(ctx, x, weight, bias, call):
        _lib.require_gpu(x, weight)
        stride, padding = call.stride, call.padding
        xc = x.detach().float().contiguous()
        n, c, h, w_ = xc.shape
        k, _, r, s = weight.shape
        ho = (h + 2 * padding[0] - (r - 1) - 1) // stride[0] + 1
        wo = (w_ + 2 * padding[1] - (s - 1) - 1) // stride[1] + 1
        kk = r * s * c
        kp = _pad_to(kk)
        key = (r, s, stride[0], padding[0], kp, x._version, x.data_ptr())
        hit = getattr(x, "_diga_xcol", None)
        cur = torch.cuda.current_stream(x.device)
        if hit is not None and hit[0] == key:
            xcol = hit[1]
            cur.wait_event(hit[2])
            xcol.record_stream(cur)
        else:
            xcol = torch.empty((n, ho, wo, kp), dtype=torch.float32, device=x.device)
            _lib.call("diga_im2col_nchw", _lib.ptr(xc), _lib.ptr(xcol), n, c, h, w_, r, s, stride[0], padding[0], ho, wo, kp,
                      _lib.stream())
            ev = torch.cuda.Event()
            ev.record(cur)
            x._diga_xcol = (key, xcol, ev)
        w2 = _pad_last(weight.detach().permute(0, 2, 3, 1).reshape(k, 1, 1, kk).contiguous(), kp)
        out = torch.empty((n, ho, wo, k), dtype=torch.float32, device=x.device)
        b = None if bias is None else bias.detach().float().contiguous()
        _conv_launch(xcol, w2, b, out, (1, 1), (0, 0), (1, 1), _TAG_FWD, call.stats, x6_ok=False, infer=call.infer)
        ctx.save_for_backward(xcol)
        ctx.geom = (k, c, r, s, kk, kp, bias is not None, weight.stride())
        return out.permute(0, 3, 1, 2)

    @staticmethod
    def backward(ctx, grad_out):
        (xcol,) = ctx.saved_tensors
        k, c, r, s, kk, kp, has_bias, w_strides = ctx.geom
        if ctx.needs_input_grad[0]:
            raise NotImplementedError("the stem conv path does not produce a gradient wrt its (image) input")
        n, ho, wo, _ = xcol.shape
        gy = grad_out.permute(0, 2, 3, 1)
        if not gy.is_contiguous():
            gy = gy.contiguous()
        kq = _pad_to(k)
        gyp = _pad_last(gy, kq)
        dw = db = None
        if ctx.needs_input_grad[1]:
            dwp = torch.empty((kq, 1, 1, kp), dtype=torch.float32, device=xcol.device)
            path = _wgrad_plan(n, ho, wo, kp, kq, 1, 1, (1, 1), (0, 0), (1, 1), ho, wo, stem=True)
            _wgrad_launch(path, gyp, xcol, dwp, 1, 1, (1, 1), (0, 0), (1, 1))
            dw = torch.empty_strided((k, c, r, s), w_strides, dtype=torch.float32, device=xcol.device)
            dw.copy_(dwp[:k, 0, 0, :kk].reshape(k, r, s, c).permute(0, 3, 1, 2))
        if has_bias and ctx.needs_input_grad[2]:
            db = _bias_grad(gy)
        return None, dw, db, None


def _set_mask(epi, box, xn, cp):
    if not box["has_res"]:
        epi.mask_y, epi.mask_ld = None, 0
    elif box.get("mask_bits") is not None:
        epi.mask_y, epi.mask_ld = None, 0
        epi.mask_bits, epi.mask_bits_ld = _lib.ptr(box["mask_bits"]), cp // 8
    else:
        epi.mask_y, epi.mask_ld = _lib.ptr(xn), cp


class _Conv2dFn(torch.autograd.Function):
    @staticmethod
    def forward(ctx, x, weight, bias, call):
        _lib.require_gpu(x, weight)
        stride, padding, dilation, stats, uses, twin_box, x_is_twin, dy_is_twin, bn_box, opts, chain, infer = call
        if x_is_twin:
            xt = x.detach().permute(0, 2, 3, 1)
            if not (xt.is_contiguous() and xt.dtype == torch.float32):
                raise RuntimeError("DigaConv2d: a twin-only input must be a dense NHWC float32-shaped buffer")
            twin_box = [xt.reshape(-1).view(torch.uint8)]
        if opts is not None and any(opts) and (torch.is_grad_enabled() and (x.requires_grad or weight.requires_grad)):
            raise RuntimeError("DigaConv2d: folded reflect padding / upsampling / tanh are inference-only (no backward)")
        xn = x.detach().permute(0, 2, 3, 1)
        n, hi, wi, _ = xn.shape
        k, c, r, s = weight.shape
        cp = _pad_to(c)
        up = int(opts[1]) if opts is not None else 0
        ho = ((hi << up) + 2 * padding[0] - dilation[0] * (r - 1) - 1) // stride[0] + 1
        wo = ((wi << up) + 2 * padding[1] - dilation[1] * (s - 1) - 1) // stride[1] + 1
        wino_stats = isinstance(stats, tuple)
        if wino_stats:
            stats = stats[0]
        path = _plan(n, hi, wi, cp, k, r, s, stride, (-padding[0], -padding[1]), dilation, ho, wo, _TAG_FWD,
                     None if stats is None else "records" if wino_stats else "chunks", opts=opts, infer=infer is not None,
                     shared=twin_box is not None, must_twin=bool(x_is_twin),
                     keep=ctx.needs_input_grad[1])
        in_place = (cp == c and not x_is_twin and bn_box is None and chain is None and path.family == "x6ls"
                    and _nhwc_ld(xn) is not None)
        if not in_place and (not xn.is_contiguous() or xn.dtype != torch.float32):
            xn = xn.contiguous().float()
        xn = _pad_last(xn, cp)
        w = weight.detach().permute(0, 2, 3, 1)
        if not w.is_contiguous():
            w = w.contiguous()
        w = _pad_last(w, cp)
        out = torch.empty((n, ho, wo, k), dtype=torch.float32, device=x.device)
        b = None if bias is None else bias.detach().float().contiguous()
        keep_v = [None] if path.variant == "keep" else None
        x_twin = _conv_launch(xn, w, b, out, stride, (-padding[0], -padding[1]), dilation, _TAG_FWD, stats, twin_box, opts=opts,
                              keep_v=keep_v, infer=infer, path=path)
        ctx.wino_v = keep_v[0] if keep_v is not None else None
        ctx.max_tile = config.active().winograd_max_tile
        ctx.save_for_backward(xn, w)
        ctx.x_twin = x_twin if (path.math != 2 and ctx.needs_input_grad[1] and k >= 256 and k % 8 == 0 and cp == c) else None
        ctx.x_trip = x_twin if (path.math == 2 and ctx.needs_input_grad[1]) else None
        ctx.dy_is_twin = bool(dy_is_twin)
        if dy_is_twin and ctx.x_twin is None and ctx.needs_input_grad[1]:
            raise RuntimeError("DigaConv2d: twin_grad=True on a layer whose weight gradient is not on the twin kernel")
        if x_is_twin and (x_twin is None or (ctx.needs_input_grad[1] and ctx.x_twin is None)):
            raise RuntimeError("DigaConv2d: got a twin-only input but this layer is not on the twin kernels "
                               "(check takes_twin_only_input before asking the producer for a twin)")
        ctx.geom = (stride, padding, dilation, c, bias is not None, weight.stride())
        ctx.uses = uses
        ctx.grad_view = getattr(weight, "_diga_grad_view", None) if isinstance(weight, nn.Parameter) else None
        ctx.weight_param = weight if ctx.grad_view is not None else None
        ctx.math = _lib.get_conv_math()
        ctx.x_is_twin = bool(x_is_twin)
        ctx.bn_box = None
        if (bn_box is not None and ctx.needs_input_grad[0] and stride == (1, 1) and cp == c and c % 4 == 0
                and "claimed" not in bn_box and bn_box.get("rows") == n * hi * wi and bn_box.get("C") == c
                and (not bn_box["has_res"] or not x_is_twin)):
            bn_box["claimed"] = True
            bn_box["consumer_ready"] = True
            ctx.bn_box = bn_box
        ctx.chain = chain
        if chain is not None:
            if not (ctx.needs_input_grad[0] and stride == (1, 1) and cp == c and c % 4 == 0 and not x_is_twin):
                chain["disabled"] = True
            box = chain.get("box")
            if box is not None and ("claimed" in box or box.get("rows") != n * hi * wi or box.get("C") != c):
                chain["box"] = None
            elif box is not None:
                chain["box_ok"] = True
        return out.permute(0, 3, 1, 2)

    @staticmethod
    def backward(ctx, grad_out):
        xn, w = ctx.saved_tensors
        stride, padding, dilation, c_true, has_bias, w_strides = ctx.geom
        x_trip = getattr(ctx, "x_trip", None)
        if (ctx.x_is_twin or ctx.dy_is_twin or ctx.x_twin is not None or x_trip is not None) and _lib.get_conv_math() != ctx.math:
            raise RuntimeError("DigaConv2d: the conv arithmetic (_lib.set_conv_math) changed between forward and backward of a graph that "
                               "holds split-twin tensors (their bytes are only readable by the twin kernels)")
        if ctx.x_is_twin and ctx.needs_input_grad[1] and ctx.x_twin is None:
            raise RuntimeError("DigaConv2d: twin-only input saved for backward but the weight gradient is off the twin kernel")
        n, hi, wi, cp = xn.shape
        k, r, s, _ = w.shape
        gy = grad_out.permute(0, 2, 3, 1)
        if not gy.is_contiguous():
            gy = gy.contiguous()
        _, ho, wo, _ = gy.shape
        kp = _pad_to(k)
        gyp = _pad_last(gy, kp)
        dx = dw = db = None
        st = _lib.stream()
        x_twin = getattr(ctx, "x_twin", None)
        use_tw = x_twin is not None and ctx.needs_input_grad[1] and _lib.get_conv_math() == 1 and kp == k
        dy_box = [None] if use_tw else None
        wpath = _wgrad_plan(n, hi, wi, cp, kp, r, s, stride, padding, dilation, ho, wo, x_twin=use_tw)
        dm = _layer_math(r, s, kp)
        use_x6 = wpath.math == 2
        x6_ls = wpath.family in ("x6ls", "x6rs")
        if use_x6 or dm == 2:
            dy_box = [None]
        if ctx.dy_is_twin:
            if not (kp == k and _lib.get_conv_math() == 1 and cp > 64 and (use_tw or not ctx.needs_input_grad[1])):
                raise RuntimeError("DigaConv2d: twin gradient on a layer that is not on the twin kernels")
            dy_box = [gyp.reshape(-1).view(torch.uint8)]
        if ctx.needs_input_grad[0]:
            if kp == k:
                wt = torch.empty((cp, r, s, kp), dtype=torch.float32, device=w.device)
                _lib.call("diga_weight_transpose", _lib.ptr(w), _lib.ptr(wt), k, r * s, cp, st)
            else:
                wt = torch.zeros((cp, r, s, kp), dtype=torch.float32, device=w.device)
                wt[..., :k] = w.permute(3, 1, 2, 0)
            if stride == (1, 1):
                dxn = torch.empty((n, hi, wi, cp), dtype=torch.float32, device=w.device)
                epi, box = None, ctx.bn_box
                epi_chunk = _lib.lib.diga_conv2d_epi_chunk_rows(n, ho, wo, kp, hi, wi, cp, r, s, 1, 1, padding[0], padding[1],
                                                                  dm)
                chain = ctx.chain if (ctx.chain is not None and not ctx.chain.get("disabled")) else None
                last_of_chain = False
                if chain is not None:
                    if chain.get("done"):
                        raise RuntimeError("DigaConv2d: a second backward pass through convolutions that chain their input "
                                           "gradients (retain_graph) is not supported; run the forward again")
                    chain["remaining"] -= 1
                    if chain["remaining"] < 0:
                        raise RuntimeError("DigaConv2d: gradient chain ran more members than it has")
                    last_of_chain = chain["remaining"] == 0
                    if last_of_chain:
                        chain["done"] = True
                    prev = chain.get("acc")
                    cbox = chain.get("box") if (last_of_chain and chain.get("box_ok")) else None
                    if prev is not None or cbox is not None:
                        epi = _lib.BwdEpilogue()
                        epi.addend, epi.addend_ld = _lib.ptr(prev), cp
                        if cbox is not None:
                            m_rows = n * hi * wi
                            part = torch.empty(((m_rows + 63) // 64) * 2 * cp, dtype=torch.float32, device=w.device)
                            _set_mask(epi, cbox, xn, cp)
                            epi.x, epi.x_ld = _lib.ptr(cbox["x"]), cp
                            epi.relu_ab = _lib.ptr(cbox["relu_ab"]) if not cbox["has_res"] else None
                            epi.mean, epi.invstd, epi.partials = _lib.ptr(cbox["mean"]), _lib.ptr(cbox["invstd"]), _lib.ptr(part)
                            cbox["claimed"] = True
                            cbox["premasked"] = (dxn.data_ptr(), part, dxn, prev, dxn._version, epi_chunk)
                    chain["acc"] = dxn
                elif box is not None:
                    m_rows = n * hi * wi
                    part = torch.empty(((m_rows + 63) // 64) * 2 * cp, dtype=torch.float32, device=w.device)
                    add = box.pop("dres", None)
                    box["consumed"] = True
                    epi = _lib.BwdEpilogue()
                    epi.addend, epi.addend_ld = _lib.ptr(add), cp
                    _set_mask(epi, box, xn, cp)
                    epi.x, epi.x_ld = _lib.ptr(box["x"]), cp
                    epi.relu_ab = _lib.ptr(box["relu_ab"]) if not box["has_res"] else None
                    epi.mean, epi.invstd, epi.partials = _lib.ptr(box["mean"]), _lib.ptr(box["invstd"]), _lib.ptr(part)
                    box["premasked"] = (dxn.data_ptr(), part, dxn, add, dxn._version, epi_chunk)
                _conv_launch(gyp, wt, None, dxn, (1, 1), (padding[0], padding[1]), (-dilation[0], -dilation[1]),
                             _TAG_BWD_DATA, None, dy_box if (((use_tw or ctx.dy_is_twin) and cp > 64) or dm == 2) else None,
                             must_twin=ctx.dy_is_twin, epi=epi)
            elif _strided_dgrad_ok(r, s, stride, padding, dilation):
                if ctx.dy_is_twin or ctx.bn_box is not None or (ctx.chain is not None and not ctx.chain.get("disabled")):
                    raise RuntimeError("DigaConv2d: backward-data of a stride-2 multi-tap conv takes no twin gradient (twin_grad), no "
                                       "BatchNorm-backward epilogue (bn_box) and no gradient chain")
                dxn = torch.empty((n, hi, wi, cp), dtype=torch.float32, device=w.device)
                _lib.call("diga_dgrad_strided_f32", _lib.ptr(gyp), kp, _lib.ptr(wt), _lib.ptr(dxn), cp, n, hi, wi, cp, ho, wo, kp, r, s,
                          stride[0], stride[1], padding[0], padding[1], st)
                _log_path(_TAG_BWD_DATA, "f32/s2")
                direct = 2.0 * n * ho * wo * kp * r * s * cp
                _log_flops("conv_bwd_data", direct, direct)
            else:
                if (r, s) != (1, 1) or padding != (0, 0):
                    raise NotImplementedError("backward-data of strided convs is built for 1x1 without padding (any stride) and for stride "
                                              f"(2, 2), dilation (1, 1), padding < kernel; got kernel {(r, s)}, stride {tuple(stride)}, "
                                              f"padding {tuple(padding)}, dilation {tuple(dilation)}")
                dense = torch.empty((n, ho, wo, cp), dtype=torch.float32, device=w.device)
                _conv_launch(gyp, wt, None, dense, (1, 1), (0, 0), (1, 1), _TAG_BWD_DATA, twin_box=dy_box if dm == 2 else None)
                dxn = torch.zeros((n, hi, wi, cp), dtype=torch.float32, device=w.device)
                dxn[:, ::stride[0], ::stride[1]] = dense
            dx = dxn[..., :c_true].permute(0, 3, 1, 2)
            if ctx.chain is not None and not ctx.chain.get("disabled") and ctx.chain["remaining"] > 0:
                dx = None
        if ctx.needs_input_grad[1]:
            later = False
            inline = isinstance(ctx.uses, str)
            if ctx.uses is not None and not inline:
                later = ctx.uses[0] > 0
                ctx.uses[0] += 1
            gv = getattr(ctx, "grad_view", None)
            dw = gv() if (gv is not None and not later and not inline and kp == k and cp == c_true) else None
            if dw is not None:
                held = ctx.weight_param.grad
                if held is not None and held.data_ptr() == dw.data_ptr():
                    dw = None
            if dw is None or tuple(dw.stride()) != tuple(w_strides) or dw.device != w.device:
                dw = torch.empty_strided((k, c_true, r, s), w_strides, dtype=torch.float32, device=w.device)
            alias = kp == k and cp == c_true and dw.permute(0, 2, 3, 1).is_contiguous()
            dwp = dw.permute(0, 2, 3, 1) if alias else torch.empty((kp, r, s, cp), dtype=torch.float32, device=w.device)

            splits = None
            if use_tw or (use_x6 and not x6_ls):
                dy_split, x_split = dy_box[0], x_twin if use_tw else x_trip
                if dy_split is None:
                    dy_split = _make_split(gyp, kp, n * ho * wo, kp, use_x6)
                if x_split is None:
                    x_split = _make_split(xn, xn.stride(2), n * hi * wi, cp, True)
                splits = (dy_split, x_split)
            ctx.x_trip = None

            wino_v = getattr(ctx, "wino_v", None)
            ctx.wino_v = None
            if wino_v is not None and config.active().winograd_max_tile != ctx.max_tile:
                raise RuntimeError("DigaConv2d: the Winograd tile cap changed between this layer's forward and its backward "
                                   f"({ctx.max_tile} -> {config.active().winograd_max_tile}): the kept input transform has the forward's "
                                   "layout (set_conv_math(..., exact=) belongs between steps, not inside one)")

            def run():
                _wgrad_launch(wpath, gyp, xn, dwp, r, s, stride, padding, dilation, splits, wino_v)
                if not alias:
                    dw.copy_(dwp[:k, :, :, :c_true].permute(0, 3, 1, 2))

            if later:
                _lib.join_side()
            side = None if (later or inline) else _lib.side_stream(w.device)
            if side is None:
                run()
            else:
                side.wait_stream(torch.cuda.current_stream(w.device))
                with torch.cuda.stream(side):
                    run()
                dw.record_stream(side)
                _lib.release_to_side(side, (gyp, xn) + (() if alias else (dwp,)) + (splits or ()) + ((wino_v,) if wino_v is not None else ()))
        if has_bias and ctx.needs_input_grad[2]:
            db = _bias_grad(gy)
        return dx, dw, db, None


class DigaConv2d(nn.Conv2d):

    def __init__(self, *args, **kwargs):
        super().__init__(*args, **kwargs)
        if self.groups != 1 or self.padding_mode != "zeros":
            raise NotImplementedError("DigaConv2d: groups=1 and zero padding only")
        self.emit_bn_stats = False
        self._bw_seen = [0]
        self.share_twin = False
        self.weight.data = self.weight.data.contiguous(memory_format=torch.channels_last)

    def _apply(self, fn, *a, **k):
        super()._apply(fn, *a, **k)
        if self.weight.dim() == 4 and not self.weight.data.is_contiguous(memory_format=torch.channels_last):
            self.weight.data = self.weight.data.contiguous(memory_format=torch.channels_last)
        return self

    def _stem_path(self, x):
        return (self.in_channels < 8 and not x.requires_grad and tuple(self.dilation) == (1, 1)
                and self.stride[0] == self.stride[1] and self.padding[0] == self.padding[1])

    def folds_eval_bn(self, x, bn, residual=None):
        if not config.active().fold_eval_bn:
            return False
        if torch.is_grad_enabled() and (x.requires_grad or (residual is not None and residual.requires_grad) or self.weight.requires_grad
                                        or (self.bias is not None and self.bias.requires_grad)):
            return False
        if (not isinstance(bn, nn.BatchNorm2d) or bn.training or bn.running_mean is None or bn.running_var is None or not bn.affine
                or bn.num_features != self.out_channels or self.out_channels % 4 != 0):
            return False
        if self._forward_hooks or self._forward_pre_hooks or bn._forward_hooks or bn._forward_pre_hooks:
            return False
        if self.share_twin or getattr(x, "_diga_is_twin", False) or x.dim() != 4 or not x.is_cuda:
            return False
        n, _, h, w = x.shape
        r, s = self.kernel_size
        ho = (h + 2 * self.padding[0] - self.dilation[0] * (r - 1) - 1) // self.stride[0] + 1
        wo = (w + 2 * self.padding[1] - self.dilation[1] * (s - 1) - 1) // self.stride[1] + 1
        if self._stem_path(x):
            return infer_kernel(n, ho, wo, _pad_to(r * s * self.in_channels), self.out_channels, 1, 1, (1, 1), (0, 0), (1, 1), ho, wo,
                                pointwise_ok=False) is not None
        return infer_kernel(n, h, w, _pad_to(self.in_channels), self.out_channels, r, s, tuple(self.stride), tuple(self.padding),
                            tuple(self.dilation), ho, wo) is not None

    def forward(self, x, twin_grad=False, opts=None, chain=None, infer=None):
        fn = _Conv2dFn
        if self._stem_path(x):
            fn = _StemConvFn
        stride, padding, dilation = tuple(self.stride), tuple(self.padding), tuple(self.dilation)
        stats = wino_records = None
        if infer is not None:
            from diga_amd.model.norm import eval_coefficients
            if twin_grad or chain is not None or (opts is not None and any(opts)) or getattr(x, "_diga_is_twin", False):
                raise RuntimeError("DigaConv2d: infer= is a plain forward (no twin gradient, chain, options or twin input)")
            bn, residual, relu = infer
            call = _Call(stride, padding, dilation, infer=(eval_coefficients(bn), residual, bool(relu)))
        else:
            if self.emit_bn_stats and self.training and self.out_channels % 4 == 0:
                n, _, h, w = x.shape
                r, s = self.kernel_size
                cp = _pad_to(self.in_channels)
                ho = (h + 2 * padding[0] - dilation[0] * (r - 1) - 1) // stride[0] + 1
                wo = (w + 2 * padding[1] - dilation[1] * (s - 1) - 1) // stride[1] + 1
                form, path = _stats_plan(n, h, w, cp, self.out_channels, r, s, stride, padding, dilation, ho, wo, opts, fn is _Conv2dFn)
                if form == "chunks":
                    stats = torch.empty(_lib.lib.diga_conv2d_stats_floats(n, ho, wo, self.out_channels), dtype=torch.float32,
                                        device=x.device)
                elif form == "records":
                    floats, wino_records = winograd_stats_plan(n, h, w, cp, self.out_channels, r, s, stride, padding, dilation, ho, wo)
                    stats = (torch.empty(floats, dtype=torch.float32, device=x.device), "records")
            uses = None
            if torch.is_grad_enabled() and self.weight.requires_grad:
                if self._bw_seen[0] > 0:
                    self._bw_seen[0] = 0
                uses = self._bw_seen
            twin_box = None
            if self.share_twin:
                twin_box = getattr(x, "_diga_twin_box", None)
                if twin_box is None:
                    twin_box = x._diga_twin_box = [None]
            x_is_twin = bool(getattr(x, "_diga_is_twin", False))
            if x_is_twin and fn is not _Conv2dFn:
                raise RuntimeError("DigaConv2d: twin-only input on the stem path")
            bn_box = getattr(x, "_diga_bn_box", None)
            if bn_box is not None and (self.share_twin or chain is not None or fn is not _Conv2dFn or not torch.is_grad_enabled()):
                bn_box = None
            if opts is not None and any(opts):
                if fn is not _Conv2dFn or stats is not None:
                    raise RuntimeError("DigaConv2d: folded padding / upsampling / activation need the implicit-GEMM path without BN statistics")
                call = _Call(stride, padding, dilation, None, uses, twin_box, opts=tuple(int(v) for v in opts))
            else:
                if (x_is_twin or twin_grad or bn_box is not None or chain is not None) and (fn is not _Conv2dFn or (self.bias is not None and twin_grad)):
                    if chain is None:
                        raise RuntimeError("DigaConv2d: twin gradient needs a bias-free conv on the implicit-GEMM path")
                    chain["disabled"] = True
                call = _Call(stride, padding, dilation, stats, uses, twin_box, x_is_twin, bool(twin_grad), bn_box, None, chain)
        with torch.set_grad_enabled(infer is None and torch.is_grad_enabled()):
            y = fn.apply(x, self.weight, self.bias, call)
        if wino_records is not None:
            y._diga_bn_partials = (stats[0], ("records", wino_records))
        elif stats is not None:
            chunk = _lib.lib.diga_conv2d_stats_chunk_rows(n, h, w, cp, ho, wo, self.out_channels, r, s, stride[0], stride[1],
                                                          -padding[0], -padding[1], path.math)
            y._diga_bn_partials = (stats, chunk)
        return y
```

diga_amd/train_step.py:

```python
import random

import torch

from diga_amd import _lib, ddp
from diga_amd import config as _config
from diga_amd.util import loss as L
from diga_amd.util import utils as U


_STREAMS = {}
_MISMATCH_WARNING_OFF = False


def _accumulate_on_other_streams_is_intended():
    global _MISMATCH_WARNING_OFF
    if not _MISMATCH_WARNING_OFF:
        fn = getattr(torch.autograd.graph, "set_warn_on_accumulate_grad_stream_mismatch", None)
        if fn is not None:
            fn(False)
        _MISMATCH_WARNING_OFF = True


def _shared_stream(device, role):
    idx = device.index if device.index is not None else torch.cuda.current_device()
    st = _STREAMS.get((idx, role))
    if st is None:
        st = _STREAMS[(idx, role)] = torch.cuda.Stream(device=device)
    return st


def _prefetch_stream(device):
    return _shared_stream(device, "prefetch")


class DigaTrainer:
    def __init__(self, student, teacher, base_lr=2.5e-4, max_iter=80000, power=0.9, momentum=0.9,
                 weight_decay=5e-4, rng=random, distill_scale=0.5, centroid_exchange=None, graph=None, config=None):
        self.cfg = config
        cfg = self._cfg()
        self.student, self.teacher = student, teacher
        self.base_lr, self.max_iter, self.power = base_lr, max_iter, power
        self.rng = rng
        self.distill_scale = distill_scale
        self.world = ddp.world_size()
        self.centroid_exchange = centroid_exchange or cfg.centroid_exchange
        if self.centroid_exchange not in ("allgather", "allreduce"):
            raise ValueError(f"centroid_exchange must be 'allgather' or 'allreduce', not {self.centroid_exchange!r}")
        self.opt = U.DigaSGD(student.optim_parameters(base_lr), lr=base_lr, momentum=momentum,
                             weight_decay=weight_decay, grad_scale=1.0 / self.world)
        self.use_graph = cfg.step_graph if graph is None else bool(graph)
        self._g = None
        with _config.use(cfg):
            self.reducer = ddp.GradReducer([p for p in student.parameters() if p.requires_grad], overlap=not self.use_graph)
        self._side = None
        U.create_teacher_params(teacher, student)
        for p in teacher.parameters():
            p.requires_grad_(False)

    def _cfg(self):
        return self.cfg if self.cfg is not None else _config.active()

    def prefetch_classmix(self, labels):
        if not labels.is_cuda:
            return
        if getattr(self, "_pf_stream", None) is None:
            self._pf_stream = _prefetch_stream(labels.device)
            self._pf = {}
        host, ev = U.classmix_present_async(labels, self._pf_stream)
        self._pf[id(labels)] = (labels, labels._version, host, ev)
        if len(self._pf) > 4:
            self._pf.pop(next(iter(self._pf)))

    def _present(self, labels):
        pf = getattr(self, "_pf", None)
        hit = pf.pop(id(labels), None) if pf else None
        if hit is None or hit[0] is not labels or hit[1] != labels._version:
            return None
        hit[3].synchronize()
        return U.present_lists(hit[2])

    def _begin(self, it):
        self.student.train()
        U.adjust_learning_rate([self.opt], self.base_lr, it, self.max_iter, self.power)
        with torch.no_grad():
            U.update_teacher_params(self.teacher, self.student, it)

    def _teacher_async(self, *inputs):
        dev = inputs[0].device
        if not (inputs[0].is_cuda and _config.active().teacher_stream):
            with torch.no_grad():
                return [self.teacher(x)[2:4] for x in inputs]
        if self._side is None:
            self._side = _shared_stream(dev, "teacher")
        main = torch.cuda.current_stream(dev)
        self._side.wait_stream(main)
        self._teacher_events = []
        with torch.cuda.stream(self._side), torch.no_grad():
            outs = []
            for x in inputs:
                outs.append(self.teacher(x)[2:4])
                ev = torch.cuda.Event()
                ev.record(self._side)
                self._teacher_events.append(ev)
        for x in inputs:
            x.record_stream(self._side)
        self._pending_join = True
        return outs

    def _student_and_teacher(self, student_in, *teacher_in):
        where = _config.active().teacher_offset
        stage = None
        if where not in ("", "0"):
            stage = self.student
            for part in where.split("."):
                stage = getattr(stage, part, None) if not part.isdigit() else (stage[int(part)] if stage is not None and int(part) < len(stage) else None)
                if stage is None:
                    break
        if not isinstance(stage, torch.nn.Module) or not _config.active().teacher_stream or not student_in.is_cuda:
            pending = self._teacher_async(*teacher_in)
            return self.student(student_in), pending
        box = {}

        def launch(mod, inp, out):
            if "p" not in box:
                box["p"] = self._teacher_async(*teacher_in)

        handle = stage.register_forward_hook(launch)
        try:
            s_out = self.student(student_in)
        finally:
            handle.remove()
        if "p" not in box:
            box["p"] = self._teacher_async(*teacher_in)
        return s_out, box["p"]

    def _teacher_join(self, outs):
        if getattr(self, "_pending_join", False):
            main = torch.cuda.current_stream(outs[0][0].device)
            main.wait_stream(self._side)
            for pair in outs:
# ... 269 lines not shown
```

diga_amd/util/utils.py:

```python
import os
import random
import sys

import numpy as np
import torch

_pkg = os.path.dirname(os.path.dirname(os.path.abspath(__file__)))
if os.path.dirname(_pkg) not in sys.path:
    sys.path.append(os.path.dirname(_pkg))
from diga_amd import _lib

CHUNK_ELEMS = 16384


def poly_lr_scheduler_warm(base_lr, iter, warmup=1000, max_iter=80000, power=1.0):
    if iter <= warmup:
        return base_lr * (iter / warmup)
    return base_lr * ((1 - float(iter - warmup) / max_iter) ** power)


def poly_lr_scheduler(base_lr, iter, max_iter=30000, power=0.9):
    return base_lr * ((1 - float(iter) / max_iter) ** power)


# ... 37 lines not shown
        self.n_chunks = len(ct)
        self.sizes = torch.tensor(sizes, dtype=torch.int64, device=device)
        self.chunk_tensor = torch.tensor(ct, dtype=torch.int32, device=device)
        self.chunk_start = torch.tensor(cs, dtype=torch.int64, device=device)
        self._ptrs = {}

    def pointers(self, slot, tensors):
        host = [t.data_ptr() for t in tensors]
        cached = self._ptrs.get(slot)
        if cached is None or cached[0] != host:
            dev = torch.tensor(host, dtype=torch.int64, device=self.device)
            self._ptrs[slot] = (host, dev)
            return dev
        return cached[1]


def same_dense_layout(a, b):
    if a.shape != b.shape:
        return False
    if a.is_contiguous() and b.is_contiguous():
        return True
    return (a.dim() == 4 and a.is_contiguous(memory_format=torch.channels_last)
            and b.is_contiguous(memory_format=torch.channels_last))


def _check_param_lists(a, b, what):
    if len(a) != len(b):
        raise ValueError(f"{what}: {len(a)} vs {len(b)} parameters")
    for x, y in zip(a, b):
        if x.dtype != torch.float32 or y.dtype != torch.float32:
            raise TypeError(f"{what}: fp32 parameters expected")
        if not same_dense_layout(x, y):
            raise ValueError(f"{what}: parameters differ in shape or memory layout "
                             f"({tuple(x.shape)}/{x.stride()} vs {tuple(y.shape)}/{y.stride()})")
    _lib.require_gpu(*a, *b)


_ema_tables = {}


def _ema_multi(teacher_params, student_params, alpha):
    t = [p.data for p in teacher_params]
    s = [p.data for p in student_params]
    _check_param_lists(t, s, "update_teacher_params")
    key = tuple(x.data_ptr() for x in t) + tuple(x.data_ptr() for x in s)
    tab = _ema_tables.get(key)
    if tab is None:
        _ema_tables.clear()
        tab = _ema_tables[key] = TensorTables([x.numel() for x in t], t[0].device)
    tp, sp = tab.pointers("t", t), tab.pointers("s", s)
    one_minus = float(1 - alpha)
    _lib.call("diga_ema_update_multi", _lib.ptr(tp), _lib.ptr(sp), _lib.ptr(tab.sizes), _lib.ptr(tab.chunk_tensor),
              _lib.ptr(tab.chunk_start), tab.n_chunks, CHUNK_ELEMS, float(alpha), one_minus, _lib.stream())


def ema_alpha(iteration, stage0=True, mean=False, replace=False):
    if stage0:
        return min(1 - 1 / (iteration + 1), 0.999)
    if mean:
        return 0.9
    if replace:
        return 0.0
    return 0.999


def create_teacher_params(teacher, student):
    for param in teacher.parameters():
        param.detach_()
    with torch.no_grad():
        for tp, sp in zip(teacher.parameters(), student.parameters()):
            tp.data.copy_(sp.data)
    return teacher.cuda()


def update_teacher_params(teacher, student, iteration, stage0=True, mean=False, replace=False):
    alpha = ema_alpha(iteration, stage0, mean, replace)
    tflat, sflat = getattr(teacher, "flat_params", None), getattr(student, "flat_params", None)
    if tflat is not None and sflat is not None and tflat.numel() == sflat.numel():
        _lib.require_gpu(tflat, sflat)
        _lib.call("diga_ema_update_flat", _lib.ptr(tflat), _lib.ptr(sflat), tflat.numel(), float(alpha),
                  float(1 - alpha), _lib.stream())
    else:
        _ema_multi(list(teacher.parameters()), list(student.parameters()), alpha)
    return teacher


class UnNormalize(object):
    def __init__(self, mean, std):
        self.mean, self.std = mean, std

    def __call__(self, tensor):
        m = torch.as_tensor(self.mean, dtype=tensor.dtype, device=tensor.device).view(1, -1, 1, 1)
        s = torch.as_tensor(self.std, dtype=tensor.dtype, device=tensor.device).view(1, -1, 1, 1)
        return tensor * s + m


class Normalize(object):
    def __init__(self, mean, std):
        self.mean, self.std = mean, std

    def __call__(self, tensor):
        m = torch.as_tensor(self.mean, dtype=tensor.dtype, device=tensor.device).view(1, -1, 1, 1)
        s = torch.as_tensor(self.std, dtype=tensor.dtype, device=tensor.device).view(1, -1, 1, 1)
        return (tensor - m) / s


def process_label(label, class_numbers=19):
    batch, channel, w, h = label.size()
    pred1 = torch.zeros(batch, class_numbers + 1, w, h, device=label.device)
    idx = torch.where(label < class_numbers, label, torch.full_like(label, class_numbers))
    return pred1.scatter_(1, idx.long(), 1)


def classmix_present(labels):
    _lib.require_gpu(labels)
    lab = _lib.contiguous(labels, torch.int64)
    b = lab.shape[0]
    hist = torch.zeros((b, 256), dtype=torch.int32, device=lab.device)
    _lib.call("diga_label_hist256", _lib.ptr(lab), _lib.ptr(hist), b, lab[0].numel(), _lib.stream())
    present = (hist != 0).cpu().numpy()
    return [np.nonzero(present[i])[0].tolist() for i in range(b)]


class PinnedRing(object):

    def __init__(self, shape, dtype, slots=4):
        self.bufs = [torch.empty(shape, dtype=dtype, pin_memory=True) for _ in range(slots)]
        self.events = [None] * slots
        self.i = 0

    def take(self):
        i = self.i
        self.i = (i + 1) % len(self.bufs)
        if self.events[i] is not None:
            self.events[i].synchronize()
        return i, self.bufs[i]

    def mark(self, i, event):
        self.events[i] = event


_PRESENT_RINGS = {}


def classmix_present_async(labels, stream):
    _lib.require_gpu(labels)
    lab = _lib.contiguous(labels, torch.int64)
    b = lab.shape[0]
    ring = _PRESENT_RINGS.get(b)
    if ring is None:
        ring = _PRESENT_RINGS[b] = PinnedRing((b, 256), torch.bool, slots=8)
    with torch.cuda.stream(stream):
        hist = torch.zeros((b, 256), dtype=torch.int32, device=lab.device)
        _lib.call("diga_label_hist256", _lib.ptr(lab), _lib.ptr(hist), b, lab[0].numel(), _lib.stream())
        slot, host = ring.take()
        host.copy_(hist != 0, non_blocking=True)
        ev = torch.cuda.Event()
        ev.record(stream)
        ring.mark(slot, ev)
    lab.record_stream(stream)
    return host, ev


def present_lists(host):
    present = host.numpy()
    return [np.nonzero(present[i])[0].tolist() for i in range(present.shape[0])]
# ... 142 lines not shown
```

include/diga_hip.h:

```cpp
#ifndef DIGA_HIP_H
#define DIGA_HIP_H

#include <stddef.h>
#include <stdint.h>

#ifdef __cplusplus
extern "C" {
#endif
#if defined(__GNUC__)
#pragma GCC visibility push(default)
#endif

#define DIGA_ABI_VERSION 1

#define DIGA_OK 0
#define DIGA_EINVAL (-1)
#define DIGA_EALIGN (-2)
#define DIGA_EWORKSPACE (-3)

#define DIGA_IGNORE_LABEL 255

int diga_version(void);
const char* diga_last_error_string(void);

// ... 104 lines not shown
    const float* x;
    int64_t x_ld;
    const float* relu_ab;
    const float* mean;
    const float* invstd;
    float* partials;
    const unsigned char* mask_bits;
    int64_t mask_bits_ld;
} diga_bwd_epilogue_t;

int diga_conv2d_nhwc_f32_epi(const float* in, const float* wgt, float* out, int64_t N, int64_t Hi, int64_t Wi, int64_t Cin,
                             int64_t in_ld, int64_t Ho, int64_t Wo, int64_t Cout, int64_t out_ld, int64_t R, int64_t S,
                             int64_t stride_y, int64_t stride_x, int64_t off_y0, int64_t off_x0, int64_t off_dy,
                             int64_t off_dx, const diga_bwd_epilogue_t* epi, int prof_tag, void* stream);
int diga_conv2d_nhwc_bf16x3_epi(const float* in, const uint16_t* wgt_hi, const uint16_t* wgt_lo, float* out, int64_t N,
                                int64_t Hi, int64_t Wi, int64_t Cin, int64_t in_ld, int64_t Ho, int64_t Wo, int64_t Cout,
                                int64_t out_ld, int64_t R, int64_t S, int64_t stride_y, int64_t stride_x, int64_t off_y0,
                                int64_t off_x0, int64_t off_dy, int64_t off_dx, const diga_bwd_epilogue_t* epi, int prof_tag,
                                void* stream);
int diga_conv2d_nhwc_twin_epi(const void* in_twin, const void* wgt_img, float* out, int64_t N, int64_t Hi, int64_t Wi,
                              int64_t Cin, int64_t Ho, int64_t Wo, int64_t Cout, int64_t out_ld, int64_t R, int64_t S,
                              int64_t stride_y, int64_t stride_x, int64_t off_y0, int64_t off_x0, int64_t off_dy,
                              int64_t off_dx, const diga_bwd_epilogue_t* epi, int prof_tag, void* stream);

typedef struct {
    const float* ab;
    const float* residual;
    int64_t residual_ld;
    int relu;
} diga_infer_epilogue_t;

int diga_conv2d_nhwc_f32_infer(const float* in, const float* wgt, const float* bias, float* out,
                               int64_t N, int64_t Hi, int64_t Wi, int64_t Cin, int64_t in_ld,
                               int64_t Ho, int64_t Wo, int64_t Cout, int64_t out_ld, int64_t R, int64_t S,
                               int64_t stride_y, int64_t stride_x, int64_t off_y0, int64_t off_x0,
                               int64_t off_dy, int64_t off_dx, const diga_infer_epilogue_t* infer, int prof_tag, void* stream);

typedef struct diga_conv_options {
    int reflect_pad;
    int upsample_shift;
    int activation;
} diga_conv_options_t;

#define DIGA_CONV_MATH_F32 0
#define DIGA_CONV_MATH_BF16X3 1
#define DIGA_CONV_MATH_BF16X6 2

int diga_split_bf16(const float* x, uint16_t* hi, uint16_t* lo, int64_t n, void* stream);
int diga_conv2d_nhwc_bf16x3(const float* in, const uint16_t* wgt_hi, const uint16_t* wgt_lo, const float* bias, float* out,
                            int64_t N, int64_t Hi, int64_t Wi, int64_t Cin, int64_t in_ld,
                            int64_t Ho, int64_t Wo, int64_t Cout, int64_t out_ld, int64_t R, int64_t S,
                            int64_t stride_y, int64_t stride_x, int64_t off_y0, int64_t off_x0,
                            int64_t off_dy, int64_t off_dx, float* stats_partial, int prof_tag, void* stream);

int diga_make_twin(const float* x, int64_t ld, void* twin, int64_t M, int64_t C, void* stream);
size_t diga_split_bf16_image_bytes(int64_t Cout, int64_t RS, int64_t Cin);
int diga_split_bf16_image(const float* w, void* img, int64_t Cout, int64_t RS, int64_t Cin, void* stream);
int diga_conv2d_nhwc_twin(const void* in_twin, const void* wgt_img, const float* bias, float* out, int64_t N, int64_t Hi,
                          int64_t Wi, int64_t Cin, int64_t Ho, int64_t Wo, int64_t Cout, int64_t out_ld, int64_t R, int64_t S,
                          int64_t stride_y, int64_t stride_x, int64_t off_y0, int64_t off_x0, int64_t off_dy, int64_t off_dx,
                          float* stats_partial, int prof_tag, void* stream);

size_t diga_conv2d_winograd_workspace_bytes(int64_t N, int64_t H, int64_t W, int64_t Cin, int64_t Cout, int64_t dilation, int64_t tile);
size_t diga_conv2d_winograd_tile_table_bytes(int64_t N, int64_t H, int64_t W, int64_t dilation, int64_t tile);
int diga_conv2d_winograd_tile_table(void* table, int64_t N, int64_t H, int64_t W, int64_t dilation, int64_t tile, void* stream);
size_t diga_conv2d_winograd_stats_records(int64_t N, int64_t H, int64_t W, int64_t Cout, int64_t dilation, int64_t tile);
size_t diga_conv2d_winograd_stats_floats(int64_t N, int64_t H, int64_t W, int64_t Cout, int64_t dilation, int64_t tile);
int diga_conv2d_winograd_f32(const float* in, const float* wgt, const float* bias, float* out, void* workspace,
                             size_t workspace_bytes, int64_t N, int64_t H, int64_t W, int64_t Cin, int64_t in_ld, int64_t Cout,
                             int64_t out_ld, int64_t dilation, int64_t tile, int flip, float* stats_partial, const void* tile_table,
                             int prof_tag, void* stream);
int diga_conv2d_winograd_f32_opts(const float* in, const float* wgt, const float* bias, float* out, void* workspace,
                                  size_t workspace_bytes, int64_t N, int64_t H, int64_t W, int64_t Cin, int64_t in_ld, int64_t Cout,
                                  int64_t out_ld, int64_t dilation, int64_t tile, const diga_conv_options_t* opts, const void* tile_table,
                                  int prof_tag, void* stream);
int diga_conv2d_winograd_f32_epi(const float* in, const float* wgt, float* out, void* workspace, size_t workspace_bytes, int64_t N,
                                 int64_t H, int64_t W, int64_t Cin, int64_t in_ld, int64_t Cout, int64_t out_ld, int64_t dilation,
                                 int64_t tile, int flip, const diga_bwd_epilogue_t* epi, const void* tile_table, int prof_tag,
                                 void* stream);
int diga_conv2d_winograd_f32_infer(const float* in, const float* wgt, const float* bias, float* out, void* workspace,
                                   size_t workspace_bytes, int64_t N, int64_t H, int64_t W, int64_t Cin, int64_t in_ld, int64_t Cout,
                                   int64_t out_ld, int64_t dilation, int64_t tile, const diga_infer_epilogue_t* infer,
                                   const void* tile_table, int prof_tag, void* stream);
size_t diga_conv2d_wgrad_winograd_workspace_bytes(int64_t N, int64_t H, int64_t W, int64_t Cin, int64_t Cout, int64_t dilation,
                                                  int64_t tile, int v_kept );
int diga_conv2d_wgrad_winograd_f32(const float* dy, const float* x, const float* v_kept, float* dw, void* workspace,
                                   size_t workspace_bytes, int64_t N, int64_t H, int64_t W, int64_t Cin, int64_t x_ld, int64_t Cout,
                                   int64_t dy_ld, int64_t dilation, int64_t tile, const void* tile_table, void* stream);
size_t diga_conv2d_winograd_v_floats(int64_t N, int64_t H, int64_t W, int64_t Cin, int64_t dilation, int64_t tile);
int diga_conv2d_winograd_f32_keep(const float* in, const float* wgt, const float* bias, float* out, float* v_keep, void* workspace,
                                  size_t workspace_bytes, int64_t N, int64_t H, int64_t W, int64_t Cin, int64_t in_ld, int64_t Cout,
                                  int64_t out_ld, int64_t dilation, int64_t tile, float* stats_partial, const void* tile_table, int prof_tag,
                                  void* stream);

int diga_conv2d_nhwc_f32_opts(const float* in, const float* wgt, const float* bias, float* out, int64_t N, int64_t Hi, int64_t Wi,
                              int64_t Cin, int64_t in_ld, int64_t Ho, int64_t Wo, int64_t Cout, int64_t out_ld, int64_t R, int64_t S,
                              int64_t stride_y, int64_t stride_x, int64_t off_y0, int64_t off_x0, int64_t off_dy, int64_t off_dx,
                              const diga_conv_options_t* opts, int prof_tag, void* stream);
int diga_conv2d_nhwc_bf16x3_opts(const float* in, const uint16_t* wgt_hi, const uint16_t* wgt_lo, const float* bias, float* out,
                                 int64_t N, int64_t Hi, int64_t Wi, int64_t Cin, int64_t in_ld, int64_t Ho, int64_t Wo, int64_t Cout,
                                 int64_t out_ld, int64_t R, int64_t S, int64_t stride_y, int64_t stride_x, int64_t off_y0,
                                 int64_t off_x0, int64_t off_dy, int64_t off_dx, const diga_conv_options_t* opts, int prof_tag,
                                 void* stream);
int diga_conv2d_nhwc_twin_opts(const void* in_twin, const void* wgt_img, const float* bias, float* out, int64_t N, int64_t Hi,
                               int64_t Wi, int64_t Cin, int64_t Ho, int64_t Wo, int64_t Cout, int64_t out_ld, int64_t R, int64_t S,
                               int64_t stride_y, int64_t stride_x, int64_t off_y0, int64_t off_x0, int64_t off_dy, int64_t off_dx,
                               const diga_conv_options_t* opts, int prof_tag, void* stream);

size_t diga_conv2d_wgrad_workspace_bytes(int64_t N, int64_t Ho, int64_t Wo, int64_t Cout, int64_t Cin,
                                         int64_t R, int64_t S);
int diga_conv2d_wgrad_nhwc_f32(const float* dy, const float* x, float* dw, void* workspace, size_t workspace_bytes,
                               int64_t N, int64_t Hi, int64_t Wi, int64_t Cin, int64_t x_ld,
                               int64_t Ho, int64_t Wo, int64_t Cout, int64_t dy_ld, int64_t R, int64_t S,
                               int64_t stride_y, int64_t stride_x, int64_t off_y0, int64_t off_x0,
                               int64_t off_dy, int64_t off_dx, int math, void* stream);

size_t diga_conv2d_wgrad_twin_workspace_bytes(int64_t N, int64_t Ho, int64_t Wo, int64_t Cout, int64_t Cin, int64_t R, int64_t S);
int diga_conv2d_wgrad_twin(const void* dy_twin, const void* x_twin, float* dw, void* workspace, size_t workspace_bytes,
                           int64_t N, int64_t Hi, int64_t Wi, int64_t Cin, int64_t Ho, int64_t Wo, int64_t Cout, int64_t R,
                           int64_t S, int64_t stride_y, int64_t stride_x, int64_t off_y0, int64_t off_x0, int64_t off_dy,
                           int64_t off_dx, void* stream);

int diga_make_triplet(const float* x, int64_t ld, void* triplet, int64_t M, int64_t C, void* stream);
size_t diga_split_bf16x6_image_bytes(int64_t Cout, int64_t RS, int64_t Cin);
int diga_split_bf16x6_image(const float* w, void* img, int64_t Cout, int64_t RS, int64_t Cin, void* stream);
int diga_conv2d_nhwc_bf16x6(const void* in_triplet, const void* wgt_img, const float* bias, float* out, int64_t N, int64_t Hi,
                            int64_t Wi, int64_t Cin, int64_t Ho, int64_t Wo, int64_t Cout, int64_t out_ld, int64_t R, int64_t S,
                            int64_t stride_y, int64_t stride_x, int64_t off_y0, int64_t off_x0, int64_t off_dy, int64_t off_dx,
                            float* stats_partial, int prof_tag, void* stream);
int diga_conv2d_nhwc_bf16x6_epi(const void* in_triplet, const void* wgt_img, float* out, int64_t N, int64_t Hi, int64_t Wi,
                                int64_t Cin, int64_t Ho, int64_t Wo, int64_t Cout, int64_t out_ld, int64_t R, int64_t S,
                                int64_t stride_y, int64_t stride_x, int64_t off_y0, int64_t off_x0, int64_t off_dy, int64_t off_dx,
                                const diga_bwd_epilogue_t* epi, int prof_tag, void* stream);
size_t diga_conv2d_wgrad_bf16x6_workspace_bytes(int64_t N, int64_t Ho, int64_t Wo, int64_t Cout, int64_t Cin, int64_t R, int64_t S);
int diga_conv2d_wgrad_bf16x6(const void* dy_triplet, const void* x_triplet, float* dw, void* workspace, size_t workspace_bytes,
                             int64_t N, int64_t Hi, int64_t Wi, int64_t Cin, int64_t Ho, int64_t Wo, int64_t Cout, int64_t R,
                             int64_t S, int64_t stride_y, int64_t stride_x, int64_t off_y0, int64_t off_x0, int64_t off_dy,
                             int64_t off_dx, void* stream);

int diga_conv2d_nhwc_bf16x6_f32in(const float* in, int64_t in_ld, const void* wgt_img, const float* bias, float* out, int64_t N,
                                  int64_t Hi, int64_t Wi, int64_t Cin, int64_t Ho, int64_t Wo, int64_t Cout, int64_t out_ld,
                                  int64_t R, int64_t S, int64_t stride_y, int64_t stride_x, int64_t off_y0, int64_t off_x0,
                                  int64_t off_dy, int64_t off_dx, float* stats_partial, int prof_tag, void* stream);
int diga_conv2d_nhwc_bf16x6_f32in_epi(const float* in, int64_t in_ld, const void* wgt_img, float* out, int64_t N, int64_t Hi,
                                      int64_t Wi, int64_t Cin, int64_t Ho, int64_t Wo, int64_t Cout, int64_t out_ld, int64_t R,
                                      int64_t S, int64_t stride_y, int64_t stride_x, int64_t off_y0, int64_t off_x0, int64_t off_dy,
                                      int64_t off_dx, const diga_bwd_epilogue_t* epi, int prof_tag, void* stream);
int diga_conv2d_wgrad_bf16x6_f32in(const float* dy, int64_t dy_ld, const float* x, int64_t x_ld, float* dw, void* workspace,
                                   size_t workspace_bytes, int64_t N, int64_t Hi, int64_t Wi, int64_t Cin, int64_t Ho, int64_t Wo,
                                   int64_t Cout, int64_t R, int64_t S, int64_t stride_y, int64_t stride_x, int64_t off_y0,
                                   int64_t off_x0, int64_t off_dy, int64_t off_dx, void* stream);

int diga_infer_conv2d_nhwc_bf16x6(const void* in_triplet, const void* wgt_img, const float* bias, float* out, int64_t N, int64_t Hi,
                                  int64_t Wi, int64_t Cin, int64_t Ho, int64_t Wo, int64_t Cout, int64_t out_ld, int64_t R, int64_t S,
                                  int64_t stride_y, int64_t stride_x, int64_t off_y0, int64_t off_x0, int64_t off_dy, int64_t off_dx,
                                  const diga_infer_epilogue_t* infer, int prof_tag, void* stream);
int diga_infer_conv2d_nhwc_bf16x6_f32in(const float* in, int64_t in_ld, const void* wgt_img, const float* bias, float* out, int64_t N,
                                        int64_t Hi, int64_t Wi, int64_t Cin, int64_t Ho, int64_t Wo, int64_t Cout, int64_t out_ld,
                                        int64_t R, int64_t S, int64_t stride_y, int64_t stride_x, int64_t off_y0, int64_t off_x0,
                                        int64_t off_dy, int64_t off_dx, const diga_infer_epilogue_t* infer, int prof_tag,
                                        void* stream);

int diga_conv_taps_bf16x6_f32in(const float* in, int64_t in_ld, const void* wgt_img, const float* bias, float* out, int64_t N, int64_t Hi,
                                int64_t Wi, int64_t Cin, int64_t Ho, int64_t Wo, int64_t Cout, int64_t out_ld, int64_t R, int64_t S,
                                int64_t stride_y, int64_t stride_x, int64_t off_y0, int64_t off_x0, int64_t off_dy, int64_t off_dx,
                                float* stats_partial, int prof_tag, void* stream);
// ... 207 lines not shown
```

Before: 19.80 crops/s.

## Precompute Winograd weight transforms once per optimizer/EMA step in one batched kernel

Adds a PreparedWeights cache that holds Winograd U transforms (and flipped/KRSC variants for backward-data) for each conv weight. The cache is refilled with a single multi-record kernel after each optimizer step and after the teacher EMA update. Winograd convs then read the prepared U instead of transforming weights on every call. This removes the per-conv weight-transform launches at the cost of extra memory and invalidation logic keyed on epoch and data pointers. The first step runs without the cache because entries are only registered on lookup.

Result: no change. 19.76 crops/s (-0.2%).

```diff
diff --git a/diga_amd/_lib.py b/diga_amd/_lib.py
--- a/diga_amd/_lib.py
+++ b/diga_amd/_lib.py
@@ -119,6 +119,9 @@
     "diga_conv_winograd_bf16x6_opts": (INT, [P, P, P, P, P, SZ] + [I64] * 9 + [P, P, INT, P]),
     "diga_conv2d_winograd_f32_epi": (INT, [P, P, P, P, SZ] + [I64] * 9 + [INT, P, P, INT, P]),
     "diga_conv2d_winograd_f32_infer": (INT, [P, P, P, P, P, SZ] + [I64] * 9 + [P, P, INT, P]),
+    "diga_prepare_weights_blocks": (SZ, [INT, I64, I64, I64]),
+    "diga_prepare_weights_multi": (INT, [P, P, P, I64, P]),
+    "diga_winograd_f32_prepared": (INT, [P, P, P, P, P, P, SZ] + [I64] * 9 + [INT, P, P, P, P, INT, P]),
     "diga_conv2d_wgrad_winograd_workspace_bytes": (SZ, [I64] * 7 + [INT]),
     "diga_conv2d_wgrad_winograd_f32": (INT, [P, P, P, P, P, SZ] + [I64] * 9 + [P, P]),
     "diga_conv2d_winograd_v_floats": (SZ, [I64] * 6),
@@ -184,6 +187,13 @@
                 ("tiles_k", INT)]
 
 
+class WeightPrep(C.Structure):
+    _fields_ = [("src", P), ("dst", P), ("Cout", C.c_int32), ("Cin", C.c_int32), ("RS", C.c_int32), ("kind", C.c_int32)]
+
+
+PREP_TRANSPOSE, PREP_FLIP, PREP_FROM_KRSC = 0, 0x100, 0x200
+
+
 class BwdEpilogue(C.Structure):
     _fields_ = [("addend", P), ("addend_ld", I64), ("mask_y", P), ("mask_ld", I64), ("x", P), ("x_ld", I64),
                 ("relu_ab", P), ("mean", P), ("invstd", P), ("partials", P), ("mask_bits", P), ("mask_bits_ld", I64)]
diff --git a/diga_amd/config.py b/diga_amd/config.py
--- a/diga_amd/config.py
+++ b/diga_amd/config.py
@@ -38,6 +38,7 @@
     winograd_max_tile: int = 6
     winograd_keep_v: bool = True
     winograd_stats: bool = True
+    prepared_weights: bool = True
     keep_v_max_gb: float = 8.0
     keep_v_min_device_gb: float = 160.0
     conv_twin: str = "3"
@@ -83,6 +84,7 @@
         c.winograd_default_max_tile = c.winograd_max_tile = int(e("DIGA_CONV_WINOGRAD_TILE", c.winograd_default_max_tile))
         c.winograd_keep_v = _flag("DIGA_WINOGRAD_KEEP_V", c.winograd_keep_v)
         c.winograd_stats = _flag("DIGA_WINOGRAD_STATS", c.winograd_stats)
+        c.prepared_weights = _flag("DIGA_PREPARED_WEIGHTS", c.prepared_weights)
         c.keep_v_max_gb = float(e("DIGA_WINOGRAD_KEEP_V_MAX_GB", c.keep_v_max_gb))
         c.keep_v_min_device_gb = float(e("DIGA_WINOGRAD_KEEP_V_MIN_DEVICE_GB", c.keep_v_min_device_gb))
         c.conv_twin = e("DIGA_CONV_TWIN", c.conv_twin)
diff --git a/diga_amd/csrc/conv.hip b/diga_amd/csrc/conv.hip
--- a/diga_amd/csrc/conv.hip
+++ b/diga_amd/csrc/conv.hip
@@ -7,6 +7,7 @@
 
 #include "common.h"
 #include "conv_call.h"
+#include "weight_prep.h"
 
 namespace diga {
 
@@ -2193,20 +2194,7 @@
 __global__ __launch_bounds__(256) void weight_transpose_kernel(const float* __restrict__ w, float* __restrict__ wt,
                                                                int K, int RS, int C) {
     __shared__ float tile[32][33];
-    const int tap = blockIdx.z;
-    const int k0 = blockIdx.y * 32, c0 = blockIdx.x * 32;
-    const int tx = threadIdx.x & 31, ty = threadIdx.x >> 5;
-#pragma unroll
-    for (int i = 0; i < 4; ++i) {
-        const int k = k0 + ty + 8 * i, c = c0 + tx;
-        tile[ty + 8 * i][tx] = (k < K && c < C) ? w[((int64_t)k * RS + tap) * C + c] : 0.f;
-    }
-    __syncthreads();
-#pragma unroll
-    for (int i = 0; i < 4; ++i) {
-        const int c = c0 + ty + 8 * i, k = k0 + tx;
-        if (c < C && k < K) wt[((int64_t)c * RS + tap) * K + k] = tile[tx][ty + 8 * i];
-    }
+    weight_transpose_tile(w, wt, K, RS, C, blockIdx.z, blockIdx.y * 32, blockIdx.x * 32, tile);
 }
 
 static int check_conv_common(const char* who, int64_t Cin, int64_t in_ld, int64_t out_ld, int64_t Cout,
diff --git a/diga_amd/csrc/weight_prep.h b/diga_amd/csrc/weight_prep.h
--- /dev/null
+++ b/diga_amd/csrc/weight_prep.h
@@ -0,0 +1,22 @@
+#pragma once
+#include "common.h"
+
+namespace diga {
+
+__device__ __forceinline__ void weight_transpose_tile(const float* __restrict__ w, float* __restrict__ wt, int K, int RS, int C, int tap,
+                                                      int k0, int c0, float (*tile)[33]) {
+    const int tx = threadIdx.x & 31, ty = threadIdx.x >> 5;
+#pragma unroll
+    for (int i = 0; i < 4; ++i) {
+        const int k = k0 + ty + 8 * i, c = c0 + tx;
+        tile[ty + 8 * i][tx] = (k < K && c < C) ? w[((int64_t)k * RS + tap) * C + c] : 0.f;
+    }
+    __syncthreads();
+#pragma unroll
+    for (int i = 0; i < 4; ++i) {
+        const int c = c0 + ty + 8 * i, k = k0 + tx;
+        if (c < C && k < K) wt[((int64_t)c * RS + tap) * K + k] = tile[tx][ty + 8 * i];
+    }
+}
+
+}
diff --git a/diga_amd/csrc/winograd.hip b/diga_amd/csrc/winograd.hip
--- a/diga_amd/csrc/winograd.hip
+++ b/diga_amd/csrc/winograd.hip
@@ -2,6 +2,7 @@
 
 #include "common.h"
 #include "conv_call.h"
+#include "weight_prep.h"
 
 namespace diga {
 
@@ -172,11 +173,21 @@
 template <> struct Vec<4> { using In = float4; using Out = float2; using Dy = float4; using Dw = float2; static constexpr int EpiLanes = 2, EpiBlocks = 4; };
 template <> struct Vec<6> { using In = float2; using Out = float; using Dy = float2; using Dw = float2; static constexpr int EpiLanes = 2, EpiBlocks = 4; };
 
-template <int M>
-__global__ __launch_bounds__(256) void winoM_weight_kernel(const float* __restrict__ w, float* __restrict__ U, int Cout, int Cin,
-                                                           int flip) {
+template <bool KRSC>
+__device__ __forceinline__ float4 wino_weight_taps(const float* __restrict__ w, int co, int tap, int c, int Cout, int Cin) {
+    if constexpr (KRSC) {
+        const float* p = w + ((int64_t)c * 9 + tap) * Cout + co;
+        const int64_t ld = (int64_t)9 * Cout;
+        return make_float4(p[0], p[ld], p[2 * ld], p[3 * ld]);
+    } else {
+        return *reinterpret_cast<const float4*>(w + ((int64_t)co * 9 + tap) * Cin + c);
+    }
+}
+
+template <int M, bool KRSC = false>
+__device__ __forceinline__ void winoM_weight_item(const float* __restrict__ w, float* __restrict__ U, int Cout, int Cin, int flip,
+                                                  int64_t idx) {
     constexpr int A = M + 2;
-    const int64_t idx = (int64_t)blockIdx.x * 256 + threadIdx.x;
     const int c4n = Cin / 4;
     if (idx >= (int64_t)Cout * c4n) return;
     const int co = (int)(idx / c4n), c = (int)(idx - (int64_t)co * c4n) * 4;
@@ -187,7 +198,7 @@
 #pragma unroll
         for (int r = 0; r < 3; ++r) {
             const int rr = flip ? 2 - r : r, ss = flip ? 2 - s : s;
-            g[r] = *reinterpret_cast<const float4*>(w + ((int64_t)co * 9 + rr * 3 + ss) * Cin + c);
+            g[r] = wino_weight_taps<KRSC>(w, co, rr * 3 + ss, c, Cout, Cin);
         }
         float4 col[A];
         Xf<M>::g(g, col);
@@ -202,6 +213,39 @@
         Xf<M>::g(t[i], row);
 #pragma unroll
         for (int j = 0; j < A; ++j) *reinterpret_cast<float4*>(o + (A * i + j) * plane) = row[j];
+    }
+}
+template <int M>
+__global__ __launch_bounds__(256) void winoM_weight_kernel(const float* __restrict__ w, float* __restrict__ U, int Cout, int Cin,
+                                                           int flip) {
+    winoM_weight_item<M>(w, U, Cout, Cin, flip, (int64_t)blockIdx.x * 256 + threadIdx.x);
+}
+
+static inline int64_t weight_prep_blocks(int kind, int64_t Cout, int64_t Cin, int64_t RS) {
+    if ((kind & DIGA_PREP_TILE_MASK) == 0) return ceil_div(Cin, 32) * ceil_div(Cout, 32) * RS;
+    return ceil_div(Cout * (Cin / 4), 256);
+}
+__global__ __launch_bounds__(256) void weight_prep_multi_kernel(const diga_weight_prep_t* __restrict__ recs,
+                                                                const int32_t* __restrict__ chunk_record,
+                                                                const int32_t* __restrict__ chunk_block) {
+    __shared__ float tile[32][33];
+    const diga_weight_prep_t r = recs[chunk_record[blockIdx.x]];
+    const int blk = chunk_block[blockIdx.x];
+    const int m = r.kind & DIGA_PREP_TILE_MASK, flip = (r.kind & DIGA_PREP_FLIP) ? 1 : 0;
+    const bool krsc = (r.kind & DIGA_PREP_FROM_KRSC) != 0;
+    if (m == 0) {
+        const int nx = (r.Cin + 31) / 32, ny = (r.Cout + 31) / 32;
+        const int bx = blk % nx, by = (blk / nx) % ny, tap = blk / (nx * ny);
+        weight_transpose_tile(r.src, r.dst, r.Cout, r.RS, r.Cin, tap, by * 32, bx * 32, tile);
+        return;
+    }
+    const int64_t idx = (int64_t)blk * 256 + threadIdx.x;
+    if (m == 4) {
+        if (krsc) winoM_weight_item<4, true>(r.src, r.dst, r.Cout, r.Cin, flip, idx);
+        else winoM_weight_item<4>(r.src, r.dst, r.Cout, r.Cin, flip, idx);
+    } else {
+        if (krsc) winoM_weight_item<6, true>(r.src, r.dst, r.Cout, r.Cin, flip, idx);
+        else winoM_weight_item<6>(r.src, r.dst, r.Cout, r.Cin, flip, idx);
     }
 }
 
@@ -827,6 +871,7 @@
     int64_t in_ld = 0, out_ld = 0;
     int flip = 0, reflect = 0, prof_tag = 0;
     float* v_keep = nullptr;
+    const float* u_ready = nullptr;
     float* stats = nullptr;
     const diga_bwd_epilogue_t* epi = nullptr;
     const diga_infer_epilogue_t* infer = nullptr;
@@ -863,7 +908,7 @@
                  "conv2d_winograd_infer: the inference epilogue comes with the plain forward of 4x4 / 6x6 tiles");
     DIGA_REQUIRE(!reflect || (tile != 2 && !flip && !epi && dilation < H && dilation < W), DIGA_EINVAL,
                  "conv2d_winograd: reflection padding comes with the forward of 4x4 / 6x6 tiles (pad < H, W)");
-    DIGA_REQUIRE(in && wgt && out && c.workspace, DIGA_EINVAL, "conv2d_winograd: null pointer");
+    DIGA_REQUIRE(in && (wgt || c.u_ready) && out && c.workspace, DIGA_EINVAL, "conv2d_winograd: null pointer");
     DIGA_REQUIRE(N > 0 && H > 0 && W > 0 && dilation > 0 && dilation < 4096, DIGA_EINVAL, "conv2d_winograd: bad shape");
     DIGA_REQUIRE(tile_ok(tile), DIGA_EINVAL, "conv2d_winograd: tile must be 2, 4 or 6 (F(2x2,3x3) / F(4x4,3x3) / F(6x6,3x3))");
     DIGA_REQUIRE(Cin % 32 == 0 && Cout % 4 == 0 && Cout > 64 && in_ld >= Cin && in_ld % 4 == 0 && out_ld >= Cout && out_ld % 4 == 0,
@@ -881,9 +926,11 @@
     DIGA_REQUIRE(!stats || (epi == nullptr && tile != 2 && aligned16(stats)), DIGA_EINVAL,
                  "conv2d_winograd: statistics come with the forward output transform of 4x4 / 6x6 tiles (16-byte aligned buffer)");
     DIGA_REQUIRE(!tile_table || aligned16(tile_table), DIGA_EALIGN, "conv2d_winograd: tile_table must be 16-byte aligned");
+    DIGA_REQUIRE(!c.u_ready || (aligned16(c.u_ready) && !x6 && tile != 2), DIGA_EINVAL,
+                 "conv2d_winograd: a prepared U comes with the fp32 products of 4x4 / 6x6 tiles (16-byte aligned)");
     char* ws = static_cast<char*>(c.workspace);
     const int4* tab = tile_table != nullptr ? static_cast<const int4*>(tile_table) : reinterpret_cast<const int4*>(ws + l.tab);
-    float* U = reinterpret_cast<float*>(ws + l.U);
+    const float* U = c.u_ready != nullptr ? c.u_ready : reinterpret_cast<const float*>(ws + l.U);
     float* V = c.v_keep != nullptr ? c.v_keep : reinterpret_cast<float*>(ws + l.V);
     float* Mb = reinterpret_cast<float*>(ws + l.M);
     hipStream_t st = (hipStream_t)c.stream;
@@ -891,7 +938,8 @@
                    2.0 * (double)(N * H * W) * (double)Cout * 9.0 * (double)Cin);
     if (tile_table == nullptr)
         hipLaunchKernelGGL(wino_tiles_kernel, dim3((unsigned)ceil_div(g.Tp, 256)), dim3(256), 0, st, reinterpret_cast<int4*>(ws + l.tab), g);
-    with_tile(tile, [&](auto m) { launch_weight_m<decltype(m)::value>(wgt, U, Cout, Cin, flip, st); });
+    if (c.u_ready == nullptr)
+        with_tile(tile, [&](auto m) { launch_weight_m<decltype(m)::value>(wgt, reinterpret_cast<float*>(ws + l.U), Cout, Cin, flip, st); });
     launch_input(tile, in, in_ld, tab, V, g.Tp, Cin, H, W, dilation, st, reflect);
     int rc;
     if (x6) {
@@ -1011,6 +1059,44 @@
     WinoCall c;
     DIGA_FILL_WINO(c);
     c.in = in; c.in_ld = in_ld; c.wgt = wgt; c.out = out; c.out_ld = out_ld; c.flip = flip; c.epi = e; c.prof_tag = prof_tag;
+    return winograd_conv(c);
+}
+
+extern "C" size_t diga_prepare_weights_blocks(int kind, int64_t Cout, int64_t Cin, int64_t RS) {
+    const int m = kind & DIGA_PREP_TILE_MASK;
+    if (Cout <= 0 || Cin <= 0 || (kind & ~(DIGA_PREP_TILE_MASK | DIGA_PREP_FLIP | DIGA_PREP_FROM_KRSC)) != 0) return 0;
+    if (m == 0) return (kind == DIGA_PREP_TRANSPOSE && RS > 0 && RS < 65536) ? (size_t)weight_prep_blocks(kind, Cout, Cin, RS) : 0;
+    if ((m != 4 && m != 6) || RS != 9 || Cin % 4 != 0) return 0;
+    if ((kind & DIGA_PREP_FROM_KRSC) && !(kind & DIGA_PREP_FLIP)) return 0;
+    return (size_t)weight_prep_blocks(kind, Cout, Cin, RS);
+}
+
+extern "C" int diga_prepare_weights_multi(const diga_weight_prep_t* records, const int32_t* chunk_record, const int32_t* chunk_block,
+                                          int64_t n_chunks, void* stream) {
+    DIGA_REQUIRE(records && chunk_record && chunk_block, DIGA_EINVAL, "prepare_weights_multi: null table");
+    DIGA_REQUIRE(aligned16(records), DIGA_EALIGN, "prepare_weights_multi: the records must be 16-byte aligned");
+    DIGA_REQUIRE(n_chunks >= 0 && n_chunks < (1ll << 31), DIGA_EINVAL, "prepare_weights_multi: bad chunk count");
+    if (n_chunks == 0) return DIGA_OK;
+    hipLaunchKernelGGL(weight_prep_multi_kernel, dim3((unsigned)n_chunks), dim3(256), 0, (hipStream_t)stream, records, chunk_record,
+                       chunk_block);
+    return launch_status("diga_prepare_weights_multi");
+}
+
+extern "C" int diga_winograd_f32_prepared(const float* in, const float* wgt, const float* bias, float* out, float* v_keep,
+                                                 void* workspace, size_t workspace_bytes, int64_t N, int64_t H, int64_t W, int64_t Cin,
+                                                 int64_t in_ld, int64_t Cout, int64_t out_ld, int64_t dilation, int64_t tile, int flip,
+                                                 float* stats_partial, const diga_bwd_epilogue_t* e, const float* u_ready,
+                                                 const void* tile_table, int prof_tag, void* stream) {
+    DIGA_REQUIRE(u_ready != nullptr, DIGA_EINVAL, "winograd_prepared: null u_ready (the per-call forms transform the weights themselves)");
+    DIGA_REQUIRE(!v_keep || aligned16(v_keep), DIGA_EALIGN, "winograd_prepared: v_keep must be 16-byte aligned");
+    DIGA_REQUIRE(!v_keep || (!flip && !e), DIGA_EINVAL, "winograd_prepared: v_keep comes with the forward (flip = 0, no epilogue)");
+    DIGA_REQUIRE(!e || (!bias && !stats_partial), DIGA_EINVAL, "winograd_prepared: a backward epilogue takes no bias and no statistics");
+    const int rc = check_bwd_epilogue(e, Cout, "winograd_prepared");
+    if (rc) return rc;
+    WinoCall c;
+    DIGA_FILL_WINO(c);
+    c.in = in; c.in_ld = in_ld; c.wgt = wgt; c.bias = bias; c.out = out; c.out_ld = out_ld; c.flip = flip; c.v_keep = v_keep;
+    c.stats = stats_partial; c.epi = e; c.u_ready = u_ready; c.prof_tag = prof_tag;
     return winograd_conv(c);
 }
 
diff --git a/diga_amd/model/conv.py b/diga_amd/model/conv.py
--- a/diga_amd/model/conv.py
+++ b/diga_amd/model/conv.py
@@ -9,7 +9,7 @@
 _pkg = os.path.dirname(os.path.dirname(os.path.abspath(__file__)))
 if os.path.dirname(_pkg) not in sys.path:
     sys.path.append(os.path.dirname(_pkg))
-from diga_amd import _lib, config
+from diga_amd import _lib, config, prepared
 
 _TAG_FWD, _TAG_BWD_DATA = _lib.PROF_TAGS.index("conv_fwd"), _lib.PROF_TAGS.index("conv_bwd_data")
 
@@ -430,7 +430,13 @@
     return [_lib.ptr(x), _lib.ptr(w_krsc)], (), None
 
 
-def _winograd_launch(path, x, w_krsc, bias, out, d, flip, tag, stats, struct, keep_v):
+def _prepared_u(prep, weight, path, flip, cout, cin):
+    if (prep is None or path.family != "winograd" or path.x6w or path.tile not in (4, 6) or path.variant not in ("", "keep", "epi")):
+        return None
+    return prep.lookup(weight, prepared.kind_u(path.tile, flip), cout, cin, 9)
+
+
+def _winograd_launch(path, x, w_krsc, bias, out, d, flip, tag, stats, struct, keep_v, u_ready=None):
     n, hi, wi, cin = x.shape
     k, tile = out.shape[3], path.tile
     size = _lib.lib.diga_conv2d_winograd_bf16x6_workspace_bytes if path.x6w else _lib.lib.diga_conv2d_winograd_workspace_bytes
@@ -449,6 +455,11 @@
     if path.x6w:
         _lib.call(_WINOGRAD_X6, *lead, _lib.ptr(vk), *shape, flip, _lib.ptr(stats), struct, _lib.ptr(tab), tag, _lib.stream())
         return
+    if u_ready is not None:
+        _lib.call("diga_winograd_f32_prepared", _lib.ptr(x), _lib.ptr(w_krsc), _lib.ptr(None if variant == "epi" else bias),
+                  _lib.ptr(out), _lib.ptr(vk), *shape, flip, _lib.ptr(stats), struct if variant == "epi" else None, _lib.ptr(u_ready),
+                  _lib.ptr(tab), tag, _lib.stream())
+        return
     if variant == "keep":
         lead.append(_lib.ptr(vk))
     _lib.call(_ENTRY[(path.family, variant)], *lead, *shape, *((flip,) if variant in ("", "epi") else ()),
@@ -456,10 +467,10 @@
 
 
 def _conv_launch(x, w_krsc, bias, out, stride, off0, doff, tag, stats=None, twin_box=None, must_twin=False, epi=None,
-                 opts=None, keep_v=None, x6_ok=True, infer=None, path=None):
+                 opts=None, keep_v=None, x6_ok=True, infer=None, path=None, u_ready=None, taps=None):
     n, hi, wi, cin = x.shape
     _, ho, wo, k = out.shape
-    _, r, s, _ = w_krsc.shape
+    r, s = taps if w_krsc is None else w_krsc.shape[1:3]
     if path is None:
         path = _plan(n, hi, wi, cin, k, r, s, stride, off0, doff, ho, wo, tag, None if stats is None else "chunks", epi is not None,
                      opts, infer is not None, twin_box is not None, must_twin, x6_ok)
@@ -476,7 +487,7 @@
     if path.flops:
         _log_flops("conv_bwd_data" if tag == _TAG_BWD_DATA else "conv_fwd", direct, direct * path.ratio)
     if path.family in ("winograd", "winograd_reflect"):
-        _winograd_launch(path, x, w_krsc, bias, out, abs(doff[0]), 1 if doff[0] < 0 else 0, tag, stats, struct, keep_v)
+        _winograd_launch(path, x, w_krsc, bias, out, abs(doff[0]), 1 if doff[0] < 0 else 0, tag, stats, struct, keep_v, u_ready)
         return None
     lead, held, split = _operands(path, x, w_krsc, twin_box, (ho, wo, off0, opts))
     if path.family == "x6up2":
@@ -548,6 +559,7 @@
     opts: object = None
     chain: object = None
     infer: object = None
+    prep: object = None
 
 
 class _StemConvFn(torch.autograd.Function):
@@ -623,7 +635,7 @@
     @staticmethod
     def forward(ctx, x, weight, bias, call):
         _lib.require_gpu(x, weight)
-        stride, padding, dilation, stats, uses, twin_box, x_is_twin, dy_is_twin, bn_box, opts, chain, infer = call
+        stride, padding, dilation, stats, uses, twin_box, x_is_twin, dy_is_twin, bn_box, opts, chain, infer, prep = call
         if x_is_twin:
             xt = x.detach().permute(0, 2, 3, 1)
             if not (xt.is_contiguous() and xt.dtype == torch.float32):
@@ -657,8 +669,11 @@
         out = torch.empty((n, ho, wo, k), dtype=torch.float32, device=x.device)
         b = None if bias is None else bias.detach().float().contiguous()
         keep_v = [None] if path.variant == "keep" else None
+        if prep is not None and w.data_ptr() != weight.data_ptr():
+            prep = None
+        ctx.prep = (prep, weight) if prep is not None else None
         x_twin = _conv_launch(xn, w, b, out, stride, (-padding[0], -padding[1]), dilation, _TAG_FWD, stats, twin_box, opts=opts,
-                              keep_v=keep_v, infer=infer, path=path)
+                              keep_v=keep_v, infer=infer, path=path, u_ready=_prepared_u(prep, weight, path, 0, k, cp))
         ctx.wino_v = keep_v[0] if keep_v is not None else None
         ctx.max_tile = config.active().winograd_max_tile
         ctx.save_for_backward(xn, w)
@@ -728,12 +743,23 @@
                 raise RuntimeError("DigaConv2d: twin gradient on a layer that is not on the twin kernels")
             dy_box = [gyp.reshape(-1).view(torch.uint8)]
         if ctx.needs_input_grad[0]:
-            if kp == k:
-                wt = torch.empty((cp, r, s, kp), dtype=torch.float32, device=w.device)
-                _lib.call("diga_weight_transpose", _lib.ptr(w), _lib.ptr(wt), k, r * s, cp, st)
-            else:
-                wt = torch.zeros((cp, r, s, kp), dtype=torch.float32, device=w.device)
-                wt[..., :k] = w.permute(3, 1, 2, 0)
+            prep, weight = getattr(ctx, "prep", None) or (None, None)
+            if kp != k:
+                prep = None
+
+            def transposed(table=prep):
+                if table is not None:
+                    wt = table.lookup(weight, prepared.KIND_TRANSPOSE, k, cp, r * s)
+                    if wt is not None:
+                        return wt.view(cp, r, s, kp)
+                if kp == k:
+                    wt = torch.empty((cp, r, s, kp), dtype=torch.float32, device=w.device)
+                    _lib.call("diga_weight_transpose", _lib.ptr(w), _lib.ptr(wt), k, r * s, cp, st)
+                else:
+                    wt = torch.zeros((cp, r, s, kp), dtype=torch.float32, device=w.device)
+                    wt[..., :k] = w.permute(3, 1, 2, 0)
+                return wt
+
             if stride == (1, 1):
                 dxn = torch.empty((n, hi, wi, cp), dtype=torch.float32, device=w.device)
                 epi, box = None, ctx.bn_box
@@ -778,15 +804,22 @@
                     epi.relu_ab = _lib.ptr(box["relu_ab"]) if not box["has_res"] else None
                     epi.mean, epi.invstd, epi.partials = _lib.ptr(box["mean"]), _lib.ptr(box["invstd"]), _lib.ptr(part)
                     box["premasked"] = (dxn.data_ptr(), part, dxn, add, dxn._version, epi_chunk)
-                _conv_launch(gyp, wt, None, dxn, (1, 1), (padding[0], padding[1]), (-dilation[0], -dilation[1]),
-                             _TAG_BWD_DATA, None, dy_box if (((use_tw or ctx.dy_is_twin) and cp > 64) or dm == 2) else None,
-                             must_twin=ctx.dy_is_twin, epi=epi)
+                box_arg = dy_box if (((use_tw or ctx.dy_is_twin) and cp > 64) or dm == 2) else None
+                bpath = u_ready = None
+                if prep is not None:
+                    bpath = _plan(n, ho, wo, kp, cp, r, s, (1, 1), (padding[0], padding[1]), (-dilation[0], -dilation[1]), hi, wi,
+                                  _TAG_BWD_DATA, None, epi is not None, None, False, box_arg is not None, ctx.dy_is_twin)
+                    u_ready = _prepared_u(prep, weight, bpath, 1, cp, kp)
+                wino_prep = bpath is not None and bpath.family == "winograd" and not bpath.x6w and bpath.tile in (4, 6)
+                _conv_launch(gyp, None if u_ready is not None else transposed(None if wino_prep else prep), None, dxn, (1, 1), (padding[0], padding[1]),
+                             (-dilation[0], -dilation[1]), _TAG_BWD_DATA, None, box_arg, must_twin=ctx.dy_is_twin, epi=epi, path=bpath,
+                             u_ready=u_ready, taps=(r, s))
             elif _strided_dgrad_ok(r, s, stride, padding, dilation):
                 if ctx.dy_is_twin or ctx.bn_box is not None or (ctx.chain is not None and not ctx.chain.get("disabled")):
                     raise RuntimeError("DigaConv2d: backward-data of a stride-2 multi-tap conv takes no twin gradient (twin_grad), no "
                                        "BatchNorm-backward epilogue (bn_box) and no gradient chain")
                 dxn = torch.empty((n, hi, wi, cp), dtype=torch.float32, device=w.device)
-                _lib.call("diga_dgrad_strided_f32", _lib.ptr(gyp), kp, _lib.ptr(wt), _lib.ptr(dxn), cp, n, hi, wi, cp, ho, wo, kp, r, s,
+                _lib.call("diga_dgrad_strided_f32", _lib.ptr(gyp), kp, _lib.ptr(transposed()), _lib.ptr(dxn), cp, n, hi, wi, cp, ho, wo, kp, r, s,
                           stride[0], stride[1], padding[0], padding[1], st)
                 _log_path(_TAG_BWD_DATA, "f32/s2")
                 direct = 2.0 * n * ho * wo * kp * r * s * cp
@@ -797,7 +830,7 @@
                                               f"(2, 2), dilation (1, 1), padding < kernel; got kernel {(r, s)}, stride {tuple(stride)}, "
                                               f"padding {tuple(padding)}, dilation {tuple(dilation)}")
                 dense = torch.empty((n, ho, wo, cp), dtype=torch.float32, device=w.device)
-                _conv_launch(gyp, wt, None, dense, (1, 1), (0, 0), (1, 1), _TAG_BWD_DATA, twin_box=dy_box if dm == 2 else None)
+                _conv_launch(gyp, transposed(), None, dense, (1, 1), (0, 0), (1, 1), _TAG_BWD_DATA, twin_box=dy_box if dm == 2 else None)
                 dxn = torch.zeros((n, hi, wi, cp), dtype=torch.float32, device=w.device)
                 dxn[:, ::stride[0], ::stride[1]] = dense
             dx = dxn[..., :c_true].permute(0, 3, 1, 2)
@@ -953,7 +986,8 @@
                     if chain is None:
                         raise RuntimeError("DigaConv2d: twin gradient needs a bias-free conv on the implicit-GEMM path")
                     chain["disabled"] = True
-                call = _Call(stride, padding, dilation, stats, uses, twin_box, x_is_twin, bool(twin_grad), bn_box, None, chain)
+                call = _Call(stride, padding, dilation, stats, uses, twin_box, x_is_twin, bool(twin_grad), bn_box, None, chain,
+                             prep=getattr(self, "_prepared", None))
         with torch.set_grad_enabled(infer is None and torch.is_grad_enabled()):
             y = fn.apply(x, self.weight, self.bias, call)
         if wino_records is not None:
diff --git a/diga_amd/prepared.py b/diga_amd/prepared.py
--- /dev/null
+++ b/diga_amd/prepared.py
@@ -0,0 +1,115 @@
+import torch
+
+from diga_amd import _lib
+
+
+def _capturing():
+    return torch.cuda.is_available() and torch.cuda.is_current_stream_capturing()
+
+
+def _none():
+    return None
+
+
+def kind_u(tile, flip):
+    return int(tile) | ((_lib.PREP_FLIP | _lib.PREP_FROM_KRSC) if flip else 0)
+
+
+KIND_TRANSPOSE = _lib.PREP_TRANSPOSE
+
+
+class _Entry:
+    __slots__ = ("param", "kind", "dims", "buf", "blocks", "epoch", "src_ptr")
+
+    def __init__(self, param, kind, dims, buf, blocks):
+        self.param, self.kind, self.dims, self.buf, self.blocks = param, kind, dims, buf, blocks
+        self.epoch, self.src_ptr = -1, 0
+
+
+class PreparedWeights:
+    def __init__(self, enabled=True):
+        self.enabled = bool(enabled)
+        self.epoch = 0
+        self._entries = {}
+        self._wanted = {}
+        self._refused = set()
+        self._table = None
+
+    def __deepcopy__(self, memo):
+        return None
+
+    def __reduce__(self):
+        return (_none, ())
+
+    def attach(self, net):
+        from diga_amd.model.conv import DigaConv2d
+        for m in net.modules():
+            if isinstance(m, DigaConv2d):
+                m._prepared = self
+        net._diga_prepared = self
+        net.register_load_state_dict_post_hook(lambda module, incompatible: self.invalidate())
+        return self
+
+    def nbytes(self):
+        return sum(e.buf.numel() * 4 for e in self._entries.values())
+
+    def invalidate(self):
+        self.epoch += 1
+
+    def lookup(self, weight, kind, cout, cin, rs):
+        if not self.enabled or not isinstance(weight, torch.nn.Parameter) or not weight.is_leaf or weight.dtype != torch.float32:
+            return None
+        if _capturing():
+            return None
+        key = (id(weight), int(kind))
+        e = self._entries.get(key)
+        if e is None:
+            if key not in self._refused:
+                self._wanted.setdefault(key, (weight, int(kind), int(cout), int(cin), int(rs)))
+            return None
+        if e.param is not weight or e.epoch != self.epoch or e.src_ptr != weight.data_ptr() or e.dims != (cout, cin, rs):
+            return None
+        return e.buf
+
+    def refill(self):
+        self.epoch += 1
+        if not self.enabled or _capturing():
+            return
+        for key, (weight, kind, cout, cin, rs) in self._wanted.items():
+            blocks = int(_lib.lib.diga_prepare_weights_blocks(kind, cout, cin, rs))
+            if blocks <= 0:
+                self._refused.add(key)
+                continue
+            tile = kind & 0xff
+            floats = (tile + 2) ** 2 * cout * cin if tile else cout * cin * rs
+            self._entries[key] = _Entry(weight, kind, (cout, cin, rs), torch.empty(floats, dtype=torch.float32, device=weight.device), blocks)
+            self._table = None
+        self._wanted.clear()
+        for key in [k for k, e in self._entries.items()
+                    if not (e.param.dim() == 4 and e.param.permute(0, 2, 3, 1).is_contiguous() and e.param.device == e.buf.device)]:
+            del self._entries[key]
+            self._table = None
+        if not self._entries:
+            return
+        entries = list(self._entries.values())
+        ptrs = [e.param.data_ptr() for e in entries]
+        if self._table is None or self._table[0] != ptrs:
+            self._table = self._build(entries, ptrs)
+        _, recs, chunk_record, chunk_block, chunks = self._table
+        _lib.call("diga_prepare_weights_multi", _lib.ptr(recs), _lib.ptr(chunk_record), _lib.ptr(chunk_block), chunks, _lib.stream())
+        for e, p in zip(entries, ptrs):
+            e.epoch, e.src_ptr = self.epoch, p
+
+    @staticmethod
+    def _build(entries, ptrs):
+        dev = entries[0].buf.device
+        recs = (_lib.WeightPrep * len(entries))()
+        which, block = [], []
+        for i, (e, p) in enumerate(zip(entries, ptrs)):
+            cout, cin, rs = e.dims
+            recs[i] = _lib.WeightPrep(p, e.buf.data_ptr(), cout, cin, rs, e.kind)
+            which.extend([i] * e.blocks)
+            block.extend(range(e.blocks))
+        raw = torch.frombuffer(bytearray(bytes(recs)), dtype=torch.uint8).to(dev)
+        return (ptrs, raw, torch.tensor(which, dtype=torch.int32, device=dev), torch.tensor(block, dtype=torch.int32, device=dev),
+                len(which))
diff --git a/diga_amd/train_step.py b/diga_amd/train_step.py
--- a/diga_amd/train_step.py
+++ b/diga_amd/train_step.py
@@ -4,6 +4,7 @@
 
 from diga_amd import _lib, ddp
 from diga_amd import config as _config
+from diga_amd.prepared import PreparedWeights
 from diga_amd.util import loss as L
 from diga_amd.util import utils as U
 
@@ -56,6 +57,14 @@
         U.create_teacher_params(teacher, student)
         for p in teacher.parameters():
             p.requires_grad_(False)
+        on = bool(cfg.prepared_weights)
+        self.prepared_student = PreparedWeights(on).attach(student)
+        self.prepared_teacher = PreparedWeights(on).attach(teacher)
+        self.opt.register_step_post_hook(lambda *_: self.prepared_student.refill())
+
+    def invalidate_prepared(self):
+        self.prepared_student.invalidate()
+        self.prepared_teacher.invalidate()
 
     def _cfg(self):
         return self.cfg if self.cfg is not None else _config.active()
diff --git a/diga_amd/util/utils.py b/diga_amd/util/utils.py
--- a/diga_amd/util/utils.py
+++ b/diga_amd/util/utils.py
@@ -143,6 +143,9 @@
                   float(1 - alpha), _lib.stream())
     else:
         _ema_multi(list(teacher.parameters()), list(student.parameters()), alpha)
+    table = getattr(teacher, "_diga_prepared", None)
+    if table is not None:
+        table.refill()
     return teacher
 
 
diff --git a/include/diga_hip.h b/include/diga_hip.h
--- a/include/diga_hip.h
+++ b/include/diga_hip.h
@@ -210,6 +210,20 @@
                                    size_t workspace_bytes, int64_t N, int64_t H, int64_t W, int64_t Cin, int64_t in_ld, int64_t Cout,
                                    int64_t out_ld, int64_t dilation, int64_t tile, const diga_infer_epilogue_t* infer,
                                    const void* tile_table, int prof_tag, void* stream);
+enum { DIGA_PREP_TRANSPOSE = 0, DIGA_PREP_TILE_MASK = 0xff, DIGA_PREP_FLIP = 0x100, DIGA_PREP_FROM_KRSC = 0x200 };
+typedef struct {
+    const float* src;
+    float* dst;
+    int32_t Cout, Cin, RS, kind;
+} diga_weight_prep_t;
+size_t diga_prepare_weights_blocks(int kind, int64_t Cout, int64_t Cin, int64_t RS);
+int diga_prepare_weights_multi(const diga_weight_prep_t* records, const int32_t* chunk_record, const int32_t* chunk_block,
+                               int64_t n_chunks, void* stream);
+int diga_winograd_f32_prepared(const float* in, const float* wgt, const float* bias, float* out, float* v_keep, void* workspace,
+                                      size_t workspace_bytes, int64_t N, int64_t H, int64_t W, int64_t Cin, int64_t in_ld, int64_t Cout,
+                                      int64_t out_ld, int64_t dilation, int64_t tile, int flip, float* stats_partial,
+                                      const diga_bwd_epilogue_t* epi, const float* u_ready, const void* tile_table, int prof_tag,
+                                      void* stream);
 size_t diga_conv2d_wgrad_winograd_workspace_bytes(int64_t N, int64_t H, int64_t W, int64_t Cin, int64_t Cout, int64_t dilation,
                                                   int64_t tile, int v_kept );
 int diga_conv2d_wgrad_winograd_f32(const float* dy, const float* x, const float* v_kept, float* dw, void* workspace,
```
